# microsoft/MaskFlownet

Measured on NVIDIA H100. Metric: image-pairs/sec (MaskFlownet-S forward, 1024x448), higher is better.
Workload: dtype f32

## Files before the change

include/maskflow_b200.h:

```cpp
#ifndef MASKFLOW_B200_H_
#define MASKFLOW_B200_H_

#ifdef __cplusplus
extern "C" {
#endif

#define MFN_VERSION 100

#if defined(__GNUC__)
#define MFN_API __attribute__((visibility("default")))
#else
#define MFN_API
#endif

#define MFN_OK 0
#define MFN_ERR_INVALID_ARG (-1)
#define MFN_ERR_UNSUPPORTED (-2)
#define MFN_ERR_ALIGNMENT (-3)

#define MFN_CORR_AUTO 0
#define MFN_CORR_GENERIC 1
#define MFN_CORR_SIMT 2
#define MFN_CORR_MMA_BF16X3 3

#define MFN_BORDER_MXNET15 0
#define MFN_BORDER_ZERO_CORNER 1

MFN_API int mfn_version(void);
MFN_API const char* mfn_last_error(void);
MFN_API const char* mfn_last_kernel(void);
MFN_API unsigned long long mfn_launch_count(void);
MFN_API int mfn_set_tuning(const char* key, int value);

MFN_API int mfn_correlation_forward(const float* data1, const float* data2, float* out, int N, int C, int H,
                            int W, int pad_size, int kernel_size, int max_displacement, int stride1,
                            int stride2, int is_multiply, long long out_batch_stride,
                            float leaky_slope, int algo, void* stream);

MFN_API int mfn_correlation_backward(const float* grad_out, const float* out, const float* data1,
                             const float* data2, float* grad1, float* grad2, int N, int C, int H,
                             int W, int max_displacement, long long out_batch_stride,
                             float leaky_slope, void* stream);

MFN_API int mfn_deformable_conv_forward(const float* data, const float* offset, const float* weight,
                                const float* bias, float* out, int N, int C, int H, int W, int F,
                                int kernel_h, int kernel_w, int stride_h, int stride_w, int dilate_h,
                                int dilate_w, int pad_h, int pad_w, int num_group,
                                int num_deformable_group, int border_mode, void* stream);

MFN_API int mfn_deformable_conv_backward(const float* grad_out, const float* data, const float* offset,
                                 const float* weight, float* grad_data, float* grad_offset,
                                 float* grad_weight, float* grad_bias, int N, int C, int H, int W,
                                 int F, int border_mode, void* stream);

MFN_API int mfn_warp_mask_forward(const float* x, const float* flow_coarse, const float* mask_coarse,
                          const float* weight, const float* bias, const float* tradeoff, float* out,
                          float* flow_up_out, float* mask_up_out, float* conv_out, int N, int C,
                          int H, int W, int F, int upsample_factor, float flow_scale,
                          float level_stride, float leaky_slope, int border_mode, void* stream);

MFN_API int mfn_warp_mask_forward_tc(const float* x, const float* flow_coarse, const float* mask_coarse,
                                     const void* packed_weight, const float* bias, const float* tradeoff, float* out,
                                     float* flow_up_out, float* mask_up_out, float* conv_out, int N, int C, int H, int W,
                                     int F, int upsample_factor, float flow_scale, float level_stride, float leaky_slope,
                                     int border_mode, void* stream);

MFN_API long long mfn_warp_resample_workspace_bytes(int N, int F, int H, int W);
MFN_API int mfn_warp_mask_forward_resample(const float* x, const float* flow_coarse, const float* mask_coarse,
                                           const float* weight, const void* packed_weight, const float* bias,
                                           const float* tradeoff, void* workspace, float* out, float* flow_up_out,
                                           float* mask_up_out, int N, int C, int H, int W, int F, int upsample_factor,
                                           float flow_scale, float level_stride, float leaky_slope, int border_mode,
                                           void* stream);

MFN_API int mfn_warp_mask_backward(const float* grad_out, const float* out, const float* conv_out,
                           const float* x, const float* flow_up, const float* mask_up,
                           const float* weight, float* grad_x, float* grad_flow_up,
                           float* grad_mask_up, float* grad_weight, float* grad_bias,
                           float* grad_tradeoff, float* grad_conv_ws, int N, int C, int H, int W,
                           int F, float flow_scale, float level_stride, float leaky_slope,
                           int border_mode, void* stream);

MFN_API int mfn_upsample_forward(const float* in, float* out, int planes, int H, int W, int factor,
                         float scale, void* stream);
MFN_API int mfn_upsample_backward(const float* grad_out, float* grad_in, int planes, int H, int W, int factor,
                          float scale, void* stream);

MFN_API int mfn_grid_generator_warp_forward(const float* flow_xy, float* grid, int N, int H, int W,
                                    void* stream);
MFN_API int mfn_bilinear_sampler_forward(const float* data, const float* grid, float* out, int N, int C,
                                 int H, int W, int OH, int OW, void* stream);

MFN_API int mfn_grid_generator_warp_backward(const float* grad_grid, float* grad_flow, int N, int H, int W,
                                             void* stream);

MFN_API int mfn_bilinear_sampler_backward(const float* grad_out, const float* data, const float* grid,
                                          float* grad_data, float* grad_grid, int N, int C, int H, int W, int OH,
                                          int OW, void* stream);

MFN_API int mfn_image_warp_concat_forward(const float* im1, const float* im2, const float* flow_q,
                                  const float* mask_q, float* c30, float* c40, int N, int Ci, int H,
                                  int W, float flow_scale, void* stream);

MFN_API int mfn_image_warp_concat_backward(const float* grad_c40, const float* im2, const float* flow_q,
                                           const float* mask_q, float* grad_im2, float* grad_flow_up,
                                           float* grad_mask_up, int N, int Ci, int H, int W, float flow_scale,
                                           void* stream);

MFN_API long long mfn_conv3x3_packed_bytes(int Cin, int Cout);
MFN_API int mfn_conv3x3_pack_weights(const float* weight , void* packed, int Cin, int Cout,
                                     void* stream);
MFN_API int mfn_conv3x3_forward(const float* x, long long x_batch_stride, const void* packed_weight, const float* bias,
                                float* out, long long out_batch_stride, int N, int Cin, int H, int W, int Cout,
                                int dilation ,
                                float leaky_slope, void* stream);
#define MFN_CONV_OUT_NCHW 0
#define MFN_CONV_OUT_DEPTH_TO_SPACE2 1
#define MFN_CONV_OUT_LINEAR_PREFIX(k) ((k) << 8)
#define MFN_CONV_BF16 0x10
MFN_API int mfn_conv3x3_forward_ex(const float* x, long long x_batch_stride, const void* packed_weight, const float* bias,
                                   float* out, long long out_batch_stride, int N, int Cin, int H, int W, int Cout,
                                   int stride, int dilation, int out_mode, float leaky_slope, void* stream);
MFN_API long long mfn_conv3x3_workspace_bytes(int N, int Cin, int H, int W, int Cout, int stride, int dilation);
MFN_API int mfn_conv3x3_forward_ws(const float* x, long long x_batch_stride, const void* packed_weight, const float* bias,
                                   float* out, long long out_batch_stride, int N, int Cin, int H, int W, int Cout,
                                   int stride, int dilation, int out_mode, float leaky_slope, void* workspace,
                                   long long workspace_bytes, void* stream);

MFN_API int mfn_split_pack(const float* src, long long src_batch_stride, int N, int C, int H, int W, void* dst,
                           int dst_channels, int dst_c0, void* stream);
MFN_API int mfn_bf16_pack(const float* src, long long src_batch_stride, int N, int C, int H, int W, void* dst,
                          int dst_channels, int dst_c0, void* stream);
MFN_API int mfn_conv3x3_forward_split(const void* x, int x_channels, int x_c0, const void* packed_weight, const float* bias,
                                      float* out, long long out_batch_stride, void* out_split, int out_split_channels,
                                      int out_split_c0, int N, int Cin, int H, int W, int Cout, int dilation, int out_mode,
                                      float leaky_slope, void* workspace, long long workspace_bytes, void* stream);

MFN_API int mfn_preprocess_forward(const void* img1, const void* img2, int is_uint8, float* out1, float* out2,
                                   float* rgb_mean, int N, int C, int H, int W, int OH, int OW, void* stream);
MFN_API int mfn_postprocess_forward(const float* pred, float* out, int N, int channels, int Hq, int Wq, int H, int W,
                                    int flip_channels, int is_flow, void* stream);

MFN_API int mfn_flow_to_color(const float* flow_xy, unsigned char* rgb, float* rad_max, int N, int H, int W,
                              float max_radius, int bgr, void* stream);

MFN_API int mfn_flow_consistency(const float* flow_fw, const float* flow_bw, unsigned char* occ_fw, unsigned char* occ_bw,
                                 int N, int H, int W, float alpha, float beta, void* stream);

MFN_API long long mfn_interpolate_frames_workspace_bytes(int N, int H, int W);
MFN_API int mfn_interpolate_frames(const unsigned char* img0, const unsigned char* img1, const float* flow_fw,
                                   const float* flow_bw, const unsigned char* occ_fw, const unsigned char* occ_bw,
                                   unsigned char* out, void* ws, long long ws_bytes, int N, int H, int W,
                                   const float* times_host, int T, float occ_weight, void* stream);

MFN_API int mfn_warp_mask_backward_det(const float* grad_out, const float* out, const float* conv_out,
                                       const float* x, const float* flow_up, const float* mask_up,
                                       const float* weight, float* grad_x, float* grad_flow_up,
                                       float* grad_mask_up, float* grad_weight, float* grad_bias,
                                       float* grad_tradeoff, float* grad_conv_ws, int N, int C, int H, int W,
                                       int F, float flow_scale, float level_stride, float leaky_slope,
                                       int border_mode, void* det_ws, long long det_ws_bytes, void* stream);
MFN_API int mfn_deformable_conv_backward_det(const float* grad_out, const float* data, const float* offset,
                                             const float* weight, float* grad_data, float* grad_offset,
                                             float* grad_weight, float* grad_bias, int N, int C, int H, int W,
                                             int F, int border_mode, void* det_ws, long long det_ws_bytes,
                                             void* stream);
MFN_API int mfn_bilinear_sampler_backward_det(const float* grad_out, const float* data, const float* grid,
                                              float* grad_data, float* grad_grid, int N, int C, int H, int W,
                                              int OH, int OW, void* det_ws, long long det_ws_bytes, void* stream);
MFN_API int mfn_image_warp_concat_backward_det(const float* grad_c40, const float* im2, const float* flow_q,
                                               const float* mask_q, float* grad_im2, float* grad_flow_up,
                                               float* grad_mask_up, int N, int Ci, int H, int W, float flow_scale,
                                               void* det_ws, long long det_ws_bytes, void* stream);
MFN_API int mfn_preprocess_forward_det(const void* img1, const void* img2, int is_uint8, float* out1, float* out2,
                                       float* rgb_mean, int N, int C, int H, int W, int OH, int OW, void* det_ws,
                                       long long det_ws_bytes, void* stream);

MFN_API int mfn_geometry_augment_forward(const void* img1, const void* img2, int is_uint8, const float* flow, const void* mask,
                                         int mask_broadcast, const float* params, float* out_img1, float* out_img2,
                                         float* out_flow, float* out_mask, int N, int H, int W, int TH, int TW, void* stream);
MFN_API long long mfn_color_augment_workspace_bytes(int N);
MFN_API int mfn_color_augment_forward(const float* img1, const float* img2, const float* params, const float* noise1,
                                      const float* noise2, float noise_sigma, long long seed, float* out1, float* out2,
                                      void* workspace, long long workspace_bytes, int N, int H, int W, int has_gamma,
                                      void* stream);

MFN_API long long mfn_multiscale_epe_workspace_bytes(int N);
MFN_API int mfn_multiscale_epe_forward(const float* flow, const float* mask, const float* const* preds, const int* scales,
                                       const float* weights, int num_scales, float eps, float q, float* loss, float* mask_sum,
                                       void* workspace, long long workspace_bytes, int N, int H, int W, void* stream);
MFN_API int mfn_multiscale_epe_backward(const float* flow, const float* mask, const float* const* preds, const int* scales,
                                        const float* weights, int num_scales, float eps, float q, const float* grad_loss,
                                        const float* mask_sum, float* const* grad_preds, int N, int H, int W, void* stream);

MFN_API int mfn_census_loss_forward(const float* img1, const float* img2w, const unsigned char* occ, float* coef, float* vsum,
                                    float* loss, void* ws, long long ws_bytes, int N, int H, int W, void* stream);
MFN_API int mfn_census_loss_backward(const float* img1, const float* img2w, const float* coef, const float* vsum,
                                     const float* g_loss, float* g_img2w, int N, int H, int W, void* stream);
MFN_API int mfn_smoothness_loss_forward(const float* flow, const float* img, float* loss, void* ws, long long ws_bytes, int N,
                                        int H, int W, void* stream);
MFN_API int mfn_smoothness_loss_backward(const float* flow, const float* img, const float* g_loss, float* g_flow, int N,
                                         int H, int W, void* stream);

#ifdef __cplusplus
}
#endif
#endif
```

maskflownet_b200/_lib.py:

```python
from __future__ import annotations

import ctypes
import os
import subprocess

_HERE = os.path.dirname(os.path.abspath(__file__))
SO_PATH = os.environ.get("MFN_LIB_PATH") or os.path.join(_HERE, "libmaskflow_b200.so")
_lib = None

_f = ctypes.c_void_p
_i = ctypes.c_int
_ll = ctypes.c_longlong
_fl = ctypes.c_float

SIGNATURES = {
    "mfn_correlation_forward": [_f, _f, _f, _i, _i, _i, _i, _i, _i, _i, _i, _i, _i, _ll, _fl, _i, _f],
    "mfn_correlation_backward": [_f, _f, _f, _f, _f, _f, _i, _i, _i, _i, _i, _ll, _fl, _f],
    "mfn_deformable_conv_forward": [_f, _f, _f, _f, _f] + [_i] * 16 + [_f],
    "mfn_deformable_conv_backward": [_f] * 8 + [_i] * 6 + [_f],
    "mfn_warp_mask_forward": [_f] * 10 + [_i] * 6 + [_fl, _fl, _fl, _i, _f],
    "mfn_warp_mask_forward_tc": [_f] * 10 + [_i] * 6 + [_fl, _fl, _fl, _i, _f],
    "mfn_warp_mask_forward_resample": [_f] * 11 + [_i] * 6 + [_fl, _fl, _fl, _i, _f],
    "mfn_warp_mask_backward": [_f] * 14 + [_i] * 5 + [_fl, _fl, _fl, _i, _f],
    "mfn_upsample_forward": [_f, _f, _i, _i, _i, _i, _fl, _f],
    "mfn_upsample_backward": [_f, _f, _i, _i, _i, _i, _fl, _f],
    "mfn_grid_generator_warp_forward": [_f, _f, _i, _i, _i, _f],
    "mfn_bilinear_sampler_forward": [_f, _f, _f, _i, _i, _i, _i, _i, _i, _f],
    "mfn_image_warp_concat_forward": [_f] * 6 + [_i] * 4 + [_fl, _f],
    "mfn_grid_generator_warp_backward": [_f, _f, _i, _i, _i, _f],
    "mfn_bilinear_sampler_backward": [_f] * 5 + [_i] * 6 + [_f],
    "mfn_image_warp_concat_backward": [_f] * 7 + [_i] * 4 + [_fl, _f],
    "mfn_preprocess_forward": [_f, _f, _i, _f, _f, _f, _i, _i, _i, _i, _i, _i, _f],
    "mfn_postprocess_forward": [_f, _f, _i, _i, _i, _i, _i, _i, _i, _i, _f],
    "mfn_flow_to_color": [_f, _f, _f, _i, _i, _i, _fl, _i, _f],
    "mfn_flow_consistency": [_f, _f, _f, _f, _i, _i, _i, _fl, _fl, _f],
    "mfn_interpolate_frames_workspace_bytes": [_i, _i, _i],
    "mfn_interpolate_frames": [_f] * 8 + [_ll, _i, _i, _i, _f, _i, _fl, _f],
    "mfn_warp_mask_backward_det": [_f] * 14 + [_i] * 5 + [_fl, _fl, _fl, _i, _f, _ll, _f],
    "mfn_deformable_conv_backward_det": [_f] * 8 + [_i] * 6 + [_f, _ll, _f],
    "mfn_bilinear_sampler_backward_det": [_f] * 5 + [_i] * 6 + [_f, _ll, _f],
    "mfn_image_warp_concat_backward_det": [_f] * 7 + [_i] * 4 + [_fl, _f, _ll, _f],
    "mfn_preprocess_forward_det": [_f, _f, _i, _f, _f, _f, _i, _i, _i, _i, _i, _i, _f, _ll, _f],
    "mfn_geometry_augment_forward": [_f, _f, _i, _f, _f, _i, _f, _f, _f, _f, _f, _i, _i, _i, _i, _i, _f],
    "mfn_color_augment_forward": [_f, _f, _f, _f, _f, _fl, _ll, _f, _f, _f, _ll, _i, _i, _i, _i, _f],
    "mfn_multiscale_epe_forward": [_f, _f, _f, _f, _f, _i, _fl, _fl, _f, _f, _f, _ll, _i, _i, _i, _f],
    "mfn_multiscale_epe_backward": [_f, _f, _f, _f, _f, _i, _fl, _fl, _f, _f, _f, _i, _i, _i, _f],
    "mfn_census_loss_forward": [_f] * 7 + [_ll, _i, _i, _i, _f],
    "mfn_census_loss_backward": [_f] * 6 + [_i, _i, _i, _f],
    "mfn_smoothness_loss_forward": [_f] * 4 + [_ll, _i, _i, _i, _f],
    "mfn_smoothness_loss_backward": [_f] * 4 + [_i, _i, _i, _f],
    "mfn_set_tuning": [ctypes.c_char_p, _i],
    "mfn_conv3x3_pack_weights": [_f, _f, _i, _i, _f],
    "mfn_conv3x3_forward": [_f, _ll, _f, _f, _f, _ll, _i, _i, _i, _i, _i, _i, _fl, _f],
    "mfn_conv3x3_forward_ex": [_f, _ll, _f, _f, _f, _ll, _i, _i, _i, _i, _i, _i, _i, _i, _fl, _f],
    "mfn_conv3x3_forward_ws": [_f, _ll, _f, _f, _f, _ll, _i, _i, _i, _i, _i, _i, _i, _i, _fl, _f, _ll, _f],
    "mfn_conv3x3_forward_split": [_f, _i, _i, _f, _f, _f, _ll, _f, _i, _i] + [_i] * 7 + [_fl, _f, _ll, _f],
    "mfn_split_pack": [_f, _ll, _i, _i, _i, _i, _f, _i, _i, _f],
    "mfn_bf16_pack": [_f, _ll, _i, _i, _i, _i, _f, _i, _i, _f],
}
RESTYPES = {"mfn_interpolate_frames_workspace_bytes": _ll}


class MaskflowError(RuntimeError):
    pass


def build(verbose: bool = False) -> str:
    cmd = ["make", "-C", os.path.join(_HERE, "csrc"), "-j8"]
    res = subprocess.run(cmd, capture_output=not verbose, text=True)
    if res.returncode != 0:
        raise MaskflowError("building libmaskflow_b200.so failed:\n" + (res.stdout or "") + (res.stderr or ""))
    return SO_PATH


def lib() -> ctypes.CDLL:
    global _lib
    if _lib is None:
        if not os.path.exists(SO_PATH):
            raise MaskflowError(
                f"{SO_PATH} is missing: run `python -c 'import __graft_entry__ as g; g.build()'` "
                "(or `make -C maskflownet_b200/csrc`).  There is no CPU / PyTorch fallback for the hot path.")
        L = ctypes.CDLL(SO_PATH)
        L.mfn_version.restype = ctypes.c_int
        L.mfn_last_error.restype = ctypes.c_char_p
        L.mfn_last_kernel.restype = ctypes.c_char_p
        L.mfn_launch_count.restype = ctypes.c_ulonglong
        L.mfn_conv3x3_packed_bytes.restype = ctypes.c_longlong
        L.mfn_conv3x3_packed_bytes.argtypes = [ctypes.c_int, ctypes.c_int]
        L.mfn_conv3x3_workspace_bytes.restype = ctypes.c_longlong
        L.mfn_conv3x3_workspace_bytes.argtypes = [ctypes.c_int] * 7
        L.mfn_color_augment_workspace_bytes.restype = ctypes.c_longlong
        L.mfn_color_augment_workspace_bytes.argtypes = [ctypes.c_int]
        L.mfn_multiscale_epe_workspace_bytes.restype = ctypes.c_longlong
        L.mfn_multiscale_epe_workspace_bytes.argtypes = [ctypes.c_int]
        L.mfn_warp_resample_workspace_bytes.restype = ctypes.c_longlong
        L.mfn_warp_resample_workspace_bytes.argtypes = [ctypes.c_int] * 4
        for name, argtypes in SIGNATURES.items():
            fn = getattr(L, name)
            fn.argtypes = argtypes
            fn.restype = RESTYPES.get(name, ctypes.c_int)
        _lib = L
        for item in filter(None, os.environ.get("MFN_TUNING", "").split(",")):
            key, _, val = item.partition("=")
            if key.strip() in ("corr_dbg", "conv_dbg"):
                raise MaskflowError(f"MFN_TUNING: {key.strip()} is a profiling switch (results invalid); set it from a tool, "
                                    "not the environment")
            if L.mfn_set_tuning(key.strip().encode(), int(val)):
                raise MaskflowError(f"MFN_TUNING: {L.mfn_last_error().decode()}")
    return _lib


def last_error() -> str:
    return lib().mfn_last_error().decode()


def last_kernel() -> str:
    return lib().mfn_last_kernel().decode()


def launch_count() -> int:
    return int(lib().mfn_launch_count())


def call(name: str, *args) -> None:
    rc = getattr(lib(), name)(*args)
    if rc != 0:
        kind = "argument/support error" if rc < 0 else "CUDA error"
        raise MaskflowError(f"{name} failed ({kind} {rc}): {last_error()}")


def set_tuning(key: str, value: int) -> None:
    call("mfn_set_tuning", key.encode(), int(value))
```

maskflownet_b200/csrc/api.cu:

```cuda
#include <atomic>
#include <cstdarg>
#include <cstdio>
#include <cstring>

#include "common.cuh"

namespace mfn {

static thread_local char g_err[512] = "";
static thread_local const char* g_kernel = "";
static std::atomic<unsigned long long> g_launches{0};

int fail(int code, const char* fmt, ...) {
  va_list ap;
  va_start(ap, fmt);
  vsnprintf(g_err, sizeof(g_err), fmt, ap);
  va_end(ap);
  return code;
}

void note_kernel(const char* name) { g_kernel = name; }

Tuning& tuning() {
  static Tuning t;
  return t;
}

int check_launch(const char* kernel_name) {
  const cudaError_t e = cudaGetLastError();
  if (e != cudaSuccess) return fail((int)e, "%s: launch failed: %s", kernel_name, cudaGetErrorString(e));
  g_kernel = kernel_name;
  g_launches.fetch_add(1, std::memory_order_relaxed);
  g_err[0] = '\0';
  return MFN_OK;
}

}

extern "C" int mfn_version(void) { return MFN_VERSION; }
extern "C" const char* mfn_last_error(void) { return mfn::g_err; }
extern "C" const char* mfn_last_kernel(void) { return mfn::g_kernel; }
extern "C" unsigned long long mfn_launch_count(void) { return mfn::g_launches.load(std::memory_order_relaxed); }

extern "C" int mfn_set_tuning(const char* key, int value) {
  if (!key) return mfn::fail(MFN_ERR_INVALID_ARG, "mfn_set_tuning: null key");
  if (!strcmp(key, "corr_grid_cap")) mfn::tuning().corr_grid_cap = value;
  else if (!strcmp(key, "corr_disable_ring")) mfn::tuning().corr_disable_ring = value;
  else if (!strcmp(key, "warp_lin")) mfn::tuning().warp_lin = value;
  else if (!strcmp(key, "corr_rb")) mfn::tuning().corr_rb = value;
  else if (!strcmp(key, "warp_lin_fch")) mfn::tuning().warp_lin_fch = value;
  else if (!strcmp(key, "conv_as")) mfn::tuning().conv_as = value;
  else if (!strcmp(key, "conv_splitk")) mfn::tuning().conv_splitk = value;
  else if (!strcmp(key, "conv_narrow")) mfn::tuning().conv_narrow = value;
  else if (!strcmp(key, "conv_tma_in")) mfn::tuning().conv_tma_in = value;
  else if (!strcmp(key, "corr_rb_twb")) mfn::tuning().corr_rb_twb = value;
  else if (!strcmp(key, "corr_rb_rows")) mfn::tuning().corr_rb_rows = value;
  else if (!strcmp(key, "corr_tma")) mfn::tuning().corr_tma = value;
  else if (!strcmp(key, "corr_ts_lo")) mfn::tuning().corr_ts_lo = value;
  else if (!strcmp(key, "corr_ts_hi")) mfn::tuning().corr_ts_hi = value;
  else if (!strcmp(key, "corr_dbg")) mfn::tuning().corr_dbg = value;
  else if (!strcmp(key, "conv_dbg")) mfn::tuning().conv_dbg = value;
  else if (!strcmp(key, "corr_ring_th")) mfn::tuning().corr_ring_th = value;
  else if (!strcmp(key, "conv_wgmma")) mfn::tuning().conv_wgmma = value;
  else if (!strcmp(key, "conv_grid_cap")) mfn::tuning().conv_grid_cap = value;
  else if (!strcmp(key, "conv_wgmma_min_w")) mfn::tuning().conv_wgmma_min_w = value;
  else return mfn::fail(MFN_ERR_INVALID_ARG, "mfn_set_tuning: unknown key '%s'", key);
  return MFN_OK;
}
```

maskflownet_b200/csrc/common.cuh:

```cuda
#pragma once
#include <cuda_runtime.h>
#include <stdint.h>

#include "../../include/maskflow_b200.h"
#include "device_caps.h"
#include "sampling.cuh"

namespace mfn {

int fail(int code, const char* fmt, ...);
int check_launch(const char* kernel_name);
void note_kernel(const char* name);

struct Tuning {
  int corr_grid_cap = 0;
  int corr_disable_ring = 0;
  int conv_wgmma = 1;
  int conv_grid_cap = 0;
  int conv_wgmma_min_w = 1;
  int corr_ring_th = 8;
  int corr_rb = 1;
  int warp_lin_fch = 0;
  int conv_as = 0;
  int conv_splitk = 1;
  int conv_narrow = 1;
  int conv_tma_in = 1;
  int corr_rb_twb = 0;
  int corr_rb_rows = 0;
  int corr_tma = 1;
  int warp_lin = 1;
  int corr_ts_lo = 0, corr_ts_hi = 0;
  int corr_dbg = 0;
  int conv_dbg = 0;
};
Tuning& tuning();

static inline cudaStream_t as_stream(void* s) { return reinterpret_cast<cudaStream_t>(s); }

#define MFN_REQUIRE(cond, code, ...)                   \
  do {                                                 \
    if (!(cond)) return ::mfn::fail(code, __VA_ARGS__); \
  } while (0)

static inline bool aligned(const void* p, size_t a) { return (reinterpret_cast<uintptr_t>(p) % a) == 0; }

static inline unsigned grid_for(long long total, int threads) {
  long long b = (total + threads - 1) / threads;
  const long long cap = (long long)kNumSMs * 16;
  return (unsigned)(b < cap ? (b > 0 ? b : 1) : cap);
}


struct SmemOptIn {
  int bytes[64] = {};
};
template <typename K>
static inline cudaError_t ensure_dyn_smem(K kernel, int bytes, SmemOptIn& st) {
  int dev = 0;
  if (cudaGetDevice(&dev) != cudaSuccess) dev = -1;
  if (dev >= 0 && dev < 64 && st.bytes[dev] >= bytes) return cudaSuccess;
  const cudaError_t e = cudaFuncSetAttribute(kernel, cudaFuncAttributeMaxDynamicSharedMemorySize, bytes);
  if (e == cudaSuccess && dev >= 0 && dev < 64) st.bytes[dev] = bytes;
  return e;
}

long long warp_lin_workspace_bytes(int N, int F, int H, int W);
int launch_warp_lin(const float* x, const float* flow_c, const float* mask_c, const float* weight, const void* packed_weight,
                    const float* bias, const float* tradeoff, void* workspace, float* out, float* fup, float* mup, int N,
                    int C, int H, int W, int F, int up, float fs, float ls, float slope, int border_mode, cudaStream_t st);

int launch_corr_rb(int md, const float* d1, const float* d2, float* out, int N, int C, int H, int W, long long obs,
                   float slope, cudaStream_t st);

int launch_corr_tma(int md, const float* d1, const float* d2, float* out, int N, int C, int H, int W, long long obs,
                    float slope, cudaStream_t st);

int det_launch_abs_max(const float* v, long long n, unsigned* bound, cudaStream_t st);
int det_launch_pixel_abs_sum_max(const float* g, int N, int F, long long HW, unsigned* bound, cudaStream_t st);
int det_launch_fixed_to_float(const unsigned long long* acc, float* out, long long n, const unsigned* bound, int nb,
                              int fanin_bits, cudaStream_t st);
int det_launch_ordered_sum(const float* part, int nparts, long long part_stride, long long elem_stride, float* out,
                           long long n, int accumulate, cudaStream_t st);
int det_check_workspace(const char* fn, const void* ws, long long bytes, long long need);

__device__ __forceinline__ float leaky(float v, float slope) { return v > 0.f ? v : v * slope; }


struct Tap {
  int h0, h1, w0, w1;
  float lh, lw;
  bool valid;
  bool c00, c01, c10, c11;
};

template <int BORDER>
__device__ __forceinline__ Tap make_tap(float h, float w, int H, int W) {
  Tap t;
  if (BORDER == MFN_BORDER_MXNET15) {
    t.valid = (h >= 0.f) && (w >= 0.f) && (h < (float)H) && (w < (float)W);
    int h0 = (int)floorf(h), w0 = (int)floorf(w);
    if (h0 >= H - 1) {
      h0 = H - 1;
      t.h1 = h0;
      t.lh = 0.f;
    } else {
      t.h1 = h0 + 1;
      t.lh = h - (float)h0;
    }
    if (w0 >= W - 1) {
      w0 = W - 1;
      t.w1 = w0;
      t.lw = 0.f;
    } else {
      t.w1 = w0 + 1;
      t.lw = w - (float)w0;
    }
    t.h0 = h0;
    t.w0 = w0;
    if (!t.valid) {
      t.h0 = t.h1 = t.w0 = t.w1 = 0;
      t.lh = t.lw = 0.f;
    }
    t.c00 = t.c01 = t.c10 = t.c11 = t.valid;
  } else {
    t.valid = (h > -1.f) && (w > -1.f) && (h < (float)H) && (w < (float)W);
    const int h0 = (int)floorf(h), w0 = (int)floorf(w);
    t.lh = h - (float)h0;
    t.lw = w - (float)w0;
    const bool hin0 = h0 >= 0, hin1 = h0 + 1 <= H - 1, win0 = w0 >= 0, win1 = w0 + 1 <= W - 1;
    t.c00 = t.valid && hin0 && win0;
    t.c01 = t.valid && hin0 && win1;
    t.c10 = t.valid && hin1 && win0;
    t.c11 = t.valid && hin1 && win1;
    t.h0 = max(min(h0, H - 1), 0);
    t.h1 = max(min(h0 + 1, H - 1), 0);
    t.w0 = max(min(w0, W - 1), 0);
    t.w1 = max(min(w0 + 1, W - 1), 0);
    if (!t.valid) t.lh = t.lw = 0.f;
  }
  return t;
}

__device__ __forceinline__ float tap_sample(const Tap& t, const float* __restrict__ plane, int W) {
  const float hh = 1.f - t.lh, hw = 1.f - t.lw;
  float v = 0.f;
  if (t.c00) v += hh * hw * __ldg(plane + (size_t)t.h0 * W + t.w0);
  if (t.c01) v += hh * t.lw * __ldg(plane + (size_t)t.h0 * W + t.w1);
  if (t.c10) v += t.lh * hw * __ldg(plane + (size_t)t.h1 * W + t.w0);
  if (t.c11) v += t.lh * t.lw * __ldg(plane + (size_t)t.h1 * W + t.w1);
  return v;
}

}
```

maskflownet_b200/csrc/conv3x3.cu:

```cuda
#include "mma_tiles.cuh"

namespace mfn {
__global__ void conv3x3_pack_kernel(const float* __restrict__ w, unsigned char* __restrict__ packed, int Cin, int Cout,
                                    int CoutP, int nChunks) {
  using namespace c3;
  const long long total = (long long)nChunks * 9 * CoutP * 16;
  for (long long i = (long long)blockIdx.x * blockDim.x + threadIdx.x; i < total; i += (long long)gridDim.x * blockDim.x) {
    const int j = (int)(i & 15);
    const int f = (int)((i >> 4) % CoutP);
    const int tap = (int)((i / (16LL * CoutP)) % 9);
    const int q = (int)(i / (16LL * CoutP * 9));
    const int c = 32 * q + 2 * j;
    float a = 0.f, b = 0.f;
    if (f < Cout) {
      if (c < Cin) a = w[((size_t)f * Cin + c) * 9 + tap];
      if (c + 1 < Cin) b = w[((size_t)f * Cin + c + 1) * 9 + tap];
    }
    uint32_t hi, lo;
    split_pair(a, b, hi, lo);
    unsigned char* tile = packed + ((size_t)q * 9 + tap) * (2 * CoutP * PXB);
    const int off = swz(f, j >> 2) + (j & 3) * 4;
    *reinterpret_cast<uint32_t*>(tile + off) = hi;
    *reinterpret_cast<uint32_t*>(tile + CoutP * PXB + off) = lo;
  }
}

template <int WC, int NTN, bool PT>
__global__ void __launch_bounds__(c3::NTHREADS, 1)
    conv3x3_mma_kernel(const float* __restrict__ x, long long x_bs, const unsigned char* __restrict__ wpack,
                       const float* __restrict__ bias, float* __restrict__ out, long long out_bs, int Cin, int H, int W,
                       int Cout, int CoutP, int nChunks, float slope, int tilesX, int tilesY, int dil, int lin_prefix) {
  using namespace c3;
  constexpr int WR = 8 / WC;
  constexpr int TROWS = PT ? WR : WR + 2;
  constexpr int HWP = PT ? TW : c3::HWP;
  constexpr int IN_LO = TROWS * HWP * PXB;
  constexpr int IN_STAGE = 2 * IN_LO;
  const int WT_LO = CoutP * PXB;
  const int WT_BYTES = 2 * WT_LO;

  extern __shared__ __align__(128) unsigned char smem[];
  unsigned char* in_s = smem;
  unsigned char* wt_s = smem + 2 * IN_STAGE;

  const int tid = threadIdx.x, warp = tid >> 5, lane = tid & 31;
  const int wr = warp / WC, wc = warp % WC;
  const int tile = blockIdx.x;
  const int tx = tile % tilesX, ty = (tile / tilesX) % tilesY, n = tile / (tilesX * tilesY);
  const int x0 = tx * TW, y0 = ty * WR;
  const size_t plane = (size_t)H * W;
  const float* xn = x + (size_t)n * x_bs;

  constexpr int U_MAIN = TROWS * 4;
  constexpr int U_HALO = PT ? 0 : ((TROWS + 3) / 4) * 4;
  constexpr int U_TOT = U_MAIN + U_HALO;
  constexpr int UPW = (U_TOT + 7) / 8;
  auto unit_geom = [&](int u, int& row, int& chunk, int& pidx, int& xx, bool& act) {
    act = u < U_TOT;
    if (u < U_MAIN) {
      row = u >> 2;
      chunk = u & 3;
      pidx = PT ? lane : HX + lane;
      xx = x0 + lane;
    } else {
      const int k = u - U_MAIN;
      row = 4 * (k >> 2) + (lane >> 3);
      chunk = k & 3;
      const int px8 = lane & 7;
      pidx = px8 < 4 ? px8 : TW + px8;
      xx = px8 < 4 ? x0 - HX + px8 : x0 + TW + (px8 - 4);
      act = act && row < TROWS;
    }
  };
  auto load_tile = [&](int q, float (&e)[UPW][8]) {
    int sy = -1, sx = 0;
    if (PT) {
      const int tap = q % 9;
      sy = (tap / 3 - 1) * dil;
      sx = (tap % 3 - 1) * dil;
      q /= 9;
    }
#pragma unroll
    for (int k = 0; k < UPW; ++k) {
      int row, chunk, pidx, xx;
      bool act;
      unit_geom(warp * UPW + k, row, chunk, pidx, xx, act);
      xx += sx;
      const int yy = y0 + sy + row;
      const bool ok = act && yy >= 0 && yy < H && xx >= 0 && xx < W;
      const int c0 = 32 * q + 8 * chunk;
      const float* p = xn + (size_t)c0 * plane + (size_t)yy * W + xx;
#pragma unroll
      for (int c = 0; c < 8; ++c) {
        e[k][c] = (ok && c0 + c < Cin) ? __ldg(p) : 0.f;
        p += plane;
      }
    }
  };
  auto store_tile = [&](int stage, const float (&e)[UPW][8]) {
#pragma unroll
    for (int k = 0; k < UPW; ++k) {
      int row, chunk, pidx, xx;
      bool act;
      unit_geom(warp * UPW + k, row, chunk, pidx, xx, act);
      if (!act) continue;
      uint4 hi, lo;
      split_pair(e[k][0], e[k][1], hi.x, lo.x);
      split_pair(e[k][2], e[k][3], hi.y, lo.y);
      split_pair(e[k][4], e[k][5], hi.z, lo.z);
      split_pair(e[k][6], e[k][7], hi.w, lo.w);
      unsigned char* dst = in_s + stage * IN_STAGE + row * (HWP * PXB) + swz(pidx, chunk);
      *reinterpret_cast<uint4*>(dst) = hi;
      *reinterpret_cast<uint4*>(dst + IN_LO) = lo;
    }
  };
  auto load_weights = [&](int it, int stage) {
    const unsigned char* src = wpack + (size_t)it * WT_BYTES;
    const uint32_t dst = smem_u32(wt_s + stage * WT_BYTES);
    for (int o = tid * 16; o < WT_BYTES; o += NTHREADS * 16) cp_async16(dst + o, src + o);
  };

  const int g = lane >> 2, j = lane & 3;
  const int l8 = lane & 7, mi = lane >> 3;
  const int swB = (l8 >> 1) & 3;
  uint32_t offB[2];
#pragma unroll
  for (int kk = 0; kk < 2; ++kk) offB[kk] = (uint32_t)((8 * (mi >> 1) + l8) * PXB + (((2 * kk + (mi & 1)) ^ swB) << 4));
  const int fbase = wc * NTN * 8;

  float acc[2][NTN][4];
#pragma unroll
  for (int mt = 0; mt < 2; ++mt)
#pragma unroll
    for (int nt = 0; nt < NTN; ++nt)
#pragma unroll
      for (int i = 0; i < 4; ++i) acc[mt][nt][i] = 0.f;

  const int nIter = nChunks * 9;
  {
    float e[UPW][8];
    load_tile(0, e);
    store_tile(0, e);
  }
  load_weights(0, 0);
  cp_async_commit();
  if (nIter > 1) load_weights(1, 1);
  cp_async_commit();

  const uint32_t in_u32 = smem_u32(in_s), wt_u32 = smem_u32(wt_s);
  float pe[UPW][8];
  for (int it = 0; it < nIter; ++it) {
    const int q = it / 9, tap = it - 9 * q;
    const int ky = tap / 3, kx = tap - 3 * ky;
    cp_async_wait<1>();
    __syncthreads();
    if (it + 2 < nIter) load_weights(it + 2, (it + 2) % WSTAGES);
    cp_async_commit();
    if (PT) {
      if (it + 1 < nIter) load_tile(it + 1, pe);
    } else {
      if (tap == 0 && q + 1 < nChunks) load_tile(q + 1, pe);
      if (tap == 8 && q + 1 < nChunks) store_tile((q + 1) & 1, pe);
    }

    const uint32_t wst = wt_u32 + (uint32_t)((it % WSTAGES) * WT_BYTES);
    const uint32_t ist = PT ? in_u32 + (uint32_t)((it & 1) * IN_STAGE + wr * (HWP * PXB))
                            : in_u32 + (uint32_t)((q & 1) * IN_STAGE + (wr + ky) * (HWP * PXB));
    const bool half_chunk = 32 * q + 16 >= Cin;
#pragma unroll
    for (int kk = 0; kk < 2; ++kk) {
      if (kk == 1 && half_chunk) break;
      uint32_t ah[2][4], al[2][4];
#pragma unroll
      for (int mt = 0; mt < 2; ++mt) {
        const int p = (PT ? 0 : HX - 1 + kx) + 16 * mt + 8 * (mi & 1) + l8;
        const uint32_t a = ist + (uint32_t)(p * PXB + (((2 * kk + (mi >> 1)) ^ ((p >> 1) & 3)) << 4));
        ldsm_x4(a, ah[mt]);
        ldsm_x4(a + IN_LO, al[mt]);
      }
#pragma unroll
      for (int nt = 0; nt < NTN; nt += 2) {
        uint32_t bh[4], bl[4];
        const uint32_t b = wst + (uint32_t)((fbase + 8 * nt) * PXB) + offB[kk];
        ldsm_x4(b, bh);
        ldsm_x4(b + WT_LO, bl);
#pragma unroll
        for (int mt = 0; mt < 2; ++mt) {
          mma_bf16(acc[mt][nt], ah[mt], bl[0], bl[1]);
          mma_bf16(acc[mt][nt], al[mt], bh[0], bh[1]);
          mma_bf16(acc[mt][nt], ah[mt], bh[0], bh[1]);
          if (nt + 1 < NTN) {
            mma_bf16(acc[mt][nt + 1], ah[mt], bl[2], bl[3]);
            mma_bf16(acc[mt][nt + 1], al[mt], bh[2], bh[3]);
            mma_bf16(acc[mt][nt + 1], ah[mt], bh[2], bh[3]);
          }
        }
      }
    }
    if (PT && it + 1 < nIter) store_tile((it + 1) & 1, pe);
  }

  const int y = y0 + wr;
  if (y >= H) return;
  float* on = out + (size_t)n * out_bs + (size_t)y * W;
#pragma unroll
  for (int nt = 0; nt < NTN; ++nt) {
#pragma unroll
    for (int i = 0; i < 4; ++i) {
      const int f = fbase + 8 * nt + 2 * j + (i & 1);
      if (f >= Cout) continue;
      const float b = bias ? __ldg(bias + f) : 0.f;
#pragma unroll
      for (int mt = 0; mt < 2; ++mt) {
        const int xx = x0 + 16 * mt + g + 8 * (i >> 1);
        if (xx < W) on[(size_t)f * plane + xx] = leaky(acc[mt][nt][i] + b, f < lin_prefix ? 1.f : slope);
      }
    }
  }
}

template <int WC, int NTN, bool PT>
static int launch_conv_impl(const float* x, long long x_bs, const unsigned char* wpack, const float* bias, float* out,
                            long long out_bs, int N, int Cin, int H, int W, int Cout, int dil, float slope, int lin_prefix,
                            cudaStream_t st) {
  using namespace c3;
  constexpr int WR = 8 / WC;
  const int CoutP = cout_pad(Cout);
  const int nChunks = (Cin + 31) / 32;
  const int tilesX = (W + TW - 1) / TW, tilesY = (H + WR - 1) / WR;
  const int in_stage = PT ? 2 * WR * TW * PXB : 2 * (WR + 2) * HWP * PXB;
  const int smem = 2 * in_stage + WSTAGES * 2 * CoutP * PXB;
  static SmemOptIn opt;
  {
    const cudaError_t e = ensure_dyn_smem(conv3x3_mma_kernel<WC, NTN, PT>, smem, opt);
    if (e != cudaSuccess) return fail((int)e, "cudaFuncSetAttribute(conv3x3_mma_kernel): %s", cudaGetErrorString(e));
  }
  const unsigned grid = (unsigned)((long long)N * tilesX * tilesY);
  conv3x3_mma_kernel<WC, NTN, PT><<<grid, NTHREADS, smem, st>>>(x, x_bs, wpack, bias, out, out_bs, Cin, H, W, Cout,
                                                               CoutP, nChunks, slope, tilesX, tilesY, dil, lin_prefix);
  return check_launch(PT ? "conv3x3_mma_kernel<per-tap tiles>" : "conv3x3_mma_kernel<halo tile>");
}

template <int WC, int NTN>
static int launch_conv(const float* x, long long x_bs, const unsigned char* wpack, const float* bias, float* out,
                       long long out_bs, int N, int Cin, int H, int W, int Cout, int dil, float slope, int lin_prefix,
                       cudaStream_t st) {
  return dil == 1 ? launch_conv_impl<WC, NTN, false>(x, x_bs, wpack, bias, out, out_bs, N, Cin, H, W, Cout, 1, slope, lin_prefix, st)
                  : launch_conv_impl<WC, NTN, true>(x, x_bs, wpack, bias, out, out_bs, N, Cin, H, W, Cout, dil, slope, lin_prefix, st);
}

long long conv3x3_sync_packed_bytes(int Cin, int Cout) {
  if (Cout > 128) return 0;
  return (long long)((Cin + 31) / 32) * 9 * 2 * c3::cout_pad(Cout) * c3::PXB;
}

}

extern "C" long long mfn_conv3x3_packed_bytes(int Cin, int Cout) {
  if (Cin <= 0 || Cout <= 0) return 0;
  return mfn::conv3x3_sync_packed_bytes(Cin, Cout) + mfn::conv3x3_wgmma_packed_bytes(Cin, Cout);
}

extern "C" int mfn_conv3x3_pack_weights(const float* weight, void* packed, int Cin, int Cout, void* stream) {
  using namespace mfn;
  MFN_REQUIRE(weight && packed, MFN_ERR_INVALID_ARG, "mfn_conv3x3_pack_weights: null pointer");
  MFN_REQUIRE(Cin > 0 && Cout > 0, MFN_ERR_INVALID_ARG, "mfn_conv3x3_pack_weights: non-positive extent");
  MFN_REQUIRE(aligned(packed, 16), MFN_ERR_ALIGNMENT, "mfn_conv3x3_pack_weights: packed buffer must be 16-byte aligned");
  MFN_REQUIRE(Cout <= 256, MFN_ERR_UNSUPPORTED, "mfn_conv3x3_pack_weights: at most 256 output channels (got %d)", Cout);
  if (Cout <= 128) {
    const int CoutP = c3::cout_pad(Cout), nChunks = (Cin + 31) / 32;
    const long long total = (long long)nChunks * 9 * CoutP * 16;
    long long blocks = (total + 255) / 256;
    if (blocks > 4096) blocks = 4096;
    conv3x3_pack_kernel<<<(unsigned)blocks, 256, 0, as_stream(stream)>>>(weight, static_cast<unsigned char*>(packed), Cin,
                                                                         Cout, CoutP, nChunks);
    const int rc = check_launch("conv3x3_pack_kernel");
    if (rc) return rc;
  }
  return conv3x3_wgmma_pack(weight, static_cast<unsigned char*>(packed) + conv3x3_sync_packed_bytes(Cin, Cout), Cin, Cout,
                           as_stream(stream));
}

extern "C" int mfn_conv3x3_forward(const float* x, long long x_batch_stride, const void* packed_weight,
                                   const float* bias, float* out, long long out_batch_stride, int N, int Cin, int H,
                                   int W, int Cout, int dilation, float leaky_slope, void* stream) {
  return mfn_conv3x3_forward_ex(x, x_batch_stride, packed_weight, bias, out, out_batch_stride, N, Cin, H, W, Cout, 1,
                                dilation, MFN_CONV_OUT_NCHW, leaky_slope, stream);
}

extern "C" int mfn_conv3x3_forward_ex(const float* x, long long x_batch_stride, const void* packed_weight,
                                      const float* bias, float* out, long long out_batch_stride, int N, int Cin, int H,
                                      int W, int Cout, int stride, int dilation, int out_mode, float leaky_slope,
                                      void* stream) {
  return mfn_conv3x3_forward_ws(x, x_batch_stride, packed_weight, bias, out, out_batch_stride, N, Cin, H, W, Cout, stride,
                                dilation, out_mode, leaky_slope, nullptr, 0, stream);
}

extern "C" long long mfn_conv3x3_workspace_bytes(int N, int Cin, int H, int W, int Cout, int stride, int dilation) {
  using namespace mfn;
  if (N <= 0 || Cin <= 0 || H <= 0 || W <= 0 || Cout <= 0 || Cout > 256 || dilation < 1 ||
      !(stride == 1 || (stride == 2 && dilation == 1)))
    return 0;
  if (!(tuning().conv_wgmma && W >= tuning().conv_wgmma_min_w) && Cout <= 128 && stride == 1) return 0;
  return conv3x3_wgmma_workspace_bytes(N, Cin, H, W, Cout, stride, dilation);
}

extern "C" int mfn_conv3x3_forward_ws(const float* x, long long x_batch_stride, const void* packed_weight,
                                      const float* bias, float* out, long long out_batch_stride, int N, int Cin, int H,
                                      int W, int Cout, int stride, int dilation, int out_mode, float leaky_slope,
                                      void* workspace, long long workspace_bytes, void* stream) {
  using namespace mfn;
  MFN_REQUIRE(workspace_bytes >= 0 && (workspace || workspace_bytes == 0) && aligned(workspace, 16), MFN_ERR_INVALID_ARG,
              "mfn_conv3x3_forward_ws: workspace must be 16-byte aligned (or null with 0 bytes)");
  MFN_REQUIRE(x && packed_weight && out, MFN_ERR_INVALID_ARG, "mfn_conv3x3_forward: null pointer");
  MFN_REQUIRE(N > 0 && Cin > 0 && H > 0 && W > 0 && Cout > 0, MFN_ERR_INVALID_ARG,
              "mfn_conv3x3_forward: non-positive extent");
  MFN_REQUIRE(Cout <= 256, MFN_ERR_UNSUPPORTED, "mfn_conv3x3_forward: at most 256 output channels (got %d)", Cout);
  MFN_REQUIRE(dilation >= 1, MFN_ERR_INVALID_ARG, "mfn_conv3x3_forward: dilation must be >= 1");
  MFN_REQUIRE(stride == 1 || (stride == 2 && dilation == 1), MFN_ERR_UNSUPPORTED,
              "mfn_conv3x3_forward: stride must be 1, or 2 with dilation 1 (got stride %d, dilation %d)", stride, dilation);
  MFN_REQUIRE(aligned(packed_weight, 16), MFN_ERR_ALIGNMENT, "mfn_conv3x3_forward: packed weights must be 16-byte aligned");
  const int bf16 = out_mode & MFN_CONV_BF16;
  out_mode &= ~MFN_CONV_BF16;
  const int lin_prefix = out_mode >> 8, mode = out_mode & 0xff;
  MFN_REQUIRE(mode == MFN_CONV_OUT_NCHW || (mode == MFN_CONV_OUT_DEPTH_TO_SPACE2 && stride == 1 && Cout % 4 == 0),
              MFN_ERR_INVALID_ARG, "mfn_conv3x3_forward: depth-to-space output needs stride 1 and Cout %% 4 == 0");
  MFN_REQUIRE(lin_prefix >= 0 && lin_prefix <= Cout && (lin_prefix == 0 || mode == MFN_CONV_OUT_NCHW), MFN_ERR_INVALID_ARG,
              "mfn_conv3x3_forward: linear prefix (out_mode >> 8 = %d) needs NCHW output and <= Cout", lin_prefix);
  const int OH = (H - 1) / stride + 1, OW = (W - 1) / stride + 1;
  const long long xbs = x_batch_stride ? x_batch_stride : (long long)Cin * H * W;
  const long long obs = out_batch_stride ? out_batch_stride : (long long)Cout * OH * OW;
  MFN_REQUIRE(xbs >= (long long)Cin * H * W && obs >= (long long)Cout * OH * OW, MFN_ERR_INVALID_ARG,
              "mfn_conv3x3_forward: batch stride smaller than the tensor");
  const unsigned char* wp = static_cast<const unsigned char*>(packed_weight);
  cudaStream_t st = as_stream(stream);
  const bool sync_ok = Cout <= 128 && stride == 1 && mode == MFN_CONV_OUT_NCHW;
  if ((tuning().conv_wgmma && W >= tuning().conv_wgmma_min_w) || !sync_ok) {
    const int rc = conv3x3_wgmma_launch(x, xbs, wp + conv3x3_sync_packed_bytes(Cin, Cout), bias, out, obs, N, Cin, H, W,
                                       Cout, stride, dilation, out_mode | bf16, leaky_slope, st, 0,
                                       static_cast<float*>(workspace), workspace_bytes);
    if (rc != -1) return rc;
    MFN_REQUIRE(sync_ok, MFN_ERR_UNSUPPORTED, "mfn_conv3x3_forward: shape fits neither kernel (Cout=%d stride=%d dilation=%d)",
                Cout, stride, dilation);
  }
  MFN_REQUIRE(!bf16, MFN_ERR_UNSUPPORTED,
              "mfn_conv3x3_forward: MFN_CONV_BF16 runs on the wgmma kernel only, and this launch would take the mma.sync "
              "kernel (tuning conv_wgmma = 0, or W = %d < conv_wgmma_min_w)", W);
  const int nt = (Cout + 7) / 8;
  if (nt <= 4) return launch_conv<1, 4>(x, xbs, wp, bias, out, obs, N, Cin, H, W, Cout, dilation, leaky_slope, lin_prefix, st);
  if (nt <= 8) return launch_conv<1, 8>(x, xbs, wp, bias, out, obs, N, Cin, H, W, Cout, dilation, leaky_slope, lin_prefix, st);
  if (nt <= 12) return launch_conv<2, 6>(x, xbs, wp, bias, out, obs, N, Cin, H, W, Cout, dilation, leaky_slope, lin_prefix, st);
  return launch_conv<2, 8>(x, xbs, wp, bias, out, obs, N, Cin, H, W, Cout, dilation, leaky_slope, lin_prefix, st);
}

extern "C" int mfn_conv3x3_forward_split(const void* x, int x_channels, int x_c0, const void* packed_weight,
                                         const float* bias, float* out, long long out_batch_stride, void* out_split,
                                         int out_split_channels, int out_split_c0, int N, int Cin, int H, int W, int Cout,
                                         int dilation, int out_mode, float leaky_slope, void* workspace,
                                         long long workspace_bytes, void* stream) {
  using namespace mfn;
  MFN_REQUIRE(workspace_bytes >= 0 && (workspace || workspace_bytes == 0) && aligned(workspace, 16), MFN_ERR_INVALID_ARG,
              "mfn_conv3x3_forward_split: workspace must be 16-byte aligned (or null with 0 bytes)");
  const int bf16 = out_mode & MFN_CONV_BF16;
  out_mode &= ~MFN_CONV_BF16;
  const int lin_prefix = out_mode >> 8, mode = out_mode & 0xff;
  MFN_REQUIRE(x && packed_weight && (out || (out_split && lin_prefix == 0)), MFN_ERR_INVALID_ARG,
              "mfn_conv3x3_forward_split: null pointer");
  MFN_REQUIRE(N > 0 && Cin > 0 && H > 0 && W > 0 && Cout > 0 && Cout <= 256 && dilation >= 1, MFN_ERR_INVALID_ARG,
              "mfn_conv3x3_forward_split: bad extent, Cout (<= 256) or dilation");
  MFN_REQUIRE(x_c0 >= 0 && x_c0 % 16 == 0 && x_c0 + Cin <= x_channels &&
                  ((x_c0 + Cin) % 16 == 0 || x_c0 + Cin == x_channels),
              MFN_ERR_INVALID_ARG,
              "mfn_conv3x3_forward_split: input slice [%d, %d) of the %d channels must start at a multiple of 16 and end "
              "at one or at the last channel", x_c0, x_c0 + Cin, x_channels);
  MFN_REQUIRE(aligned(packed_weight, 16) && aligned(x, 16), MFN_ERR_ALIGNMENT,
              "mfn_conv3x3_forward_split: packed weights and split input must be 16-byte aligned");
  MFN_REQUIRE(lin_prefix >= 0 && lin_prefix <= Cout && (lin_prefix == 0 || mode == MFN_CONV_OUT_NCHW), MFN_ERR_INVALID_ARG,
              "mfn_conv3x3_forward_split: linear prefix needs NCHW / split output and <= Cout");
  MFN_REQUIRE(mode == MFN_CONV_OUT_NCHW || (mode == MFN_CONV_OUT_DEPTH_TO_SPACE2 && Cout % 4 == 0 && !out_split),
              MFN_ERR_INVALID_ARG, "mfn_conv3x3_forward_split: depth-to-space output needs Cout %% 4 == 0 and fp32 output");
  const int Fo = out_split ? lin_prefix : (mode ? Cout / 4 : Cout), OS = mode ? 4 : 1;
  const long long obs = out_batch_stride ? out_batch_stride : (long long)Fo * H * W * OS;
  MFN_REQUIRE(obs >= (long long)Fo * H * W * OS, MFN_ERR_INVALID_ARG, "mfn_conv3x3_forward_split: batch stride too small");
  SplitIO sio;
  sio.in = x;
  sio.in_C = x_channels;
  sio.in_c0 = x_c0;
  sio.out = out_split;
  sio.out_C = out_split_channels;
  sio.out_c0 = out_split_c0;
  const unsigned char* wp = static_cast<const unsigned char*>(packed_weight);
  const int rc = conv3x3_wgmma_launch(nullptr, 0, wp + conv3x3_sync_packed_bytes(Cin, Cout), bias, out, obs, N, Cin, H, W,
                                      Cout, 1, dilation, out_mode | bf16, leaky_slope, as_stream(stream), 0,
                                      static_cast<float*>(workspace), workspace_bytes, sio);
  MFN_REQUIRE(rc != -1, MFN_ERR_UNSUPPORTED,
              "mfn_conv3x3_forward_split: unsupported (odd dilation >= 2, split output slice not 16-channel aligned "
              "after an even linear prefix, or too large)");
  return rc;
}
```

maskflownet_b200/csrc/conv3x3_wgmma.cu:

```cuda
#include <cstring>
#include <type_traits>

#include "mma_tiles.cuh"
#include "split_act.cuh"

namespace mfn {
namespace um {
constexpr int MT_WIDE = 128, MT_NARROW = 64;
inline int tile_width(int OW, int stride) {
  return tuning().conv_narrow && (OW <= MT_NARROW || (stride == 2 && tuning().conv_tma_in)) ? MT_NARROW : MT_WIDE;
}
constexpr int R = 2;
constexpr int NTHREADS = 384;
constexpr int NCONS = 8;
constexpr int NPROD = 3;
constexpr int MAX_AS = 4, MAX_WS = 24;
constexpr int MAX_RS = 4;
constexpr int BATCH = 6;
constexpr int BAR_BYTES = 1024;

__host__ __device__ inline int n_slots(int stride, int dil) { return stride == 2 ? 2 * R + 1 : (dil >= R ? 3 * R : R + 2 * dil); }
__host__ __device__ inline int row_pitch(int mt, int stride, int dil) { return stride == 2 ? 2 * mt + 1 : mt + 2 * dil; }
__host__ __device__ inline int slot_of(int r, int ky, int stride, int dil) {
  return stride == 2 ? 2 * r + ky : (dil >= R ? ky * R + r : r + ky * dil);
}
__host__ __device__ inline int tap_xoff(int mt, int kx, int stride, int dil) {
  return stride == 2 ? (kx == 1 ? 0 : (kx == 0 ? mt : mt + 1)) : kx * dil;
}
__host__ __device__ inline int band_map(int v, int n) { return v < n ? v : (v == n + 2 ? 0 : (v == n + 5 ? n - 1 : -1)); }
__host__ __device__ inline int raw_pitch(int mt, int stride) { return stride == 2 ? 2 * mt + 4 : mt + 8; }
__host__ __device__ inline int raw_channels(int stride) { return stride == 2 ? 8 : 16; }
__host__ __device__ inline int raw_stage_bytes(int nslots, int mt, int stride) {
  return raw_channels(stride) * nslots * raw_pitch(mt, stride) * 4;
}
__host__ __device__ inline int raw_ring_max(int stride) { return stride == 2 ? MAX_RS : 2; }
__host__ __device__ inline int cout_pad(int cout) { return cout <= 128 ? (cout + 15) / 16 * 16 : 256; }
__host__ __device__ inline bool fold_hi_lo(int CoutP) { return CoutP <= 64; }
__host__ __device__ inline int taps_per_stage(int CoutP) { return CoutP <= 32 ? 9 : (CoutP <= 64 ? 3 : 1); }

__device__ __forceinline__ uint64_t desc_hi(uint32_t lbo_bytes, uint32_t sbo_bytes) {
  return ((uint64_t)((lbo_bytes >> 4) & 0x3FFFu) << 16) | ((uint64_t)((sbo_bytes >> 4) & 0x3FFFu) << 32);
}
__device__ __forceinline__ void wgmma_fence() { asm volatile("wgmma.fence.sync.aligned;" ::: "memory"); }
__device__ __forceinline__ void wgmma_commit() { asm volatile("wgmma.commit_group.sync.aligned;" ::: "memory"); }
template <int N>
__device__ __forceinline__ void wgmma_wait() { asm volatile("wgmma.wait_group.sync.aligned %0;" ::"n"(N) : "memory"); }
template <int S>
__device__ __forceinline__ void fence_acc(float (&d)[S]) {
#pragma unroll
  for (int i = 0; i < S; ++i) asm volatile("" : "+f"(d[i])::"memory");
}
template <int S>
__device__ __forceinline__ void wgmma_n16(float (&d)[S], uint64_t a, uint64_t b, uint32_t scale_d) {
  static_assert(S >= 8, "accumulator too small");
  asm volatile(
      "{\n\t.reg .pred p;\n\tsetp.ne.b32 p, %10, 0;\n\t"
      "wgmma.mma_async.sync.aligned.m64n16k16.f32.bf16.bf16 {%0, %1, %2, %3, %4, %5, %6, %7}, %8, %9, p, 1, 1, 0, 0;\n\t}"
      : "+f"(d[0]), "+f"(d[1]), "+f"(d[2]), "+f"(d[3]), "+f"(d[4]), "+f"(d[5]), "+f"(d[6]), "+f"(d[7])
      : "l"(a), "l"(b), "r"(scale_d));
}
template <int S>
__device__ __forceinline__ void wgmma_n32(float (&d)[S], uint64_t a, uint64_t b, uint32_t scale_d) {
  static_assert(S >= 16, "accumulator too small");
  asm volatile(
      "{\n\t.reg .pred p;\n\tsetp.ne.b32 p, %18, 0;\n\t"
      "wgmma.mma_async.sync.aligned.m64n32k16.f32.bf16.bf16 {%0, %1, %2, %3, %4, %5, %6, %7, %8, %9, %10, %11, %12, %13, %14, %15}, %16, %17, p, 1, 1, 0, 0;\n\t}"
      : "+f"(d[0]), "+f"(d[1]), "+f"(d[2]), "+f"(d[3]), "+f"(d[4]), "+f"(d[5]), "+f"(d[6]), "+f"(d[7]), "+f"(d[8]), "+f"(d[9]), "+f"(d[10]), "+f"(d[11]), "+f"(d[12]), "+f"(d[13]), "+f"(d[14]), "+f"(d[15])
      : "l"(a), "l"(b), "r"(scale_d));
}
template <int S>
__device__ __forceinline__ void wgmma_n48(float (&d)[S], uint64_t a, uint64_t b, uint32_t scale_d) {
  static_assert(S >= 24, "accumulator too small");
  asm volatile(
      "{\n\t.reg .pred p;\n\tsetp.ne.b32 p, %26, 0;\n\t"
      "wgmma.mma_async.sync.aligned.m64n48k16.f32.bf16.bf16 {%0, %1, %2, %3, %4, %5, %6, %7, %8, %9, %10, %11, %12, %13, %14, %15, %16, %17, %18, %19, %20, %21, %22, %23}, %24, %25, p, 1, 1, 0, 0;\n\t}"
      : "+f"(d[0]), "+f"(d[1]), "+f"(d[2]), "+f"(d[3]), "+f"(d[4]), "+f"(d[5]), "+f"(d[6]), "+f"(d[7]), "+f"(d[8]), "+f"(d[9]), "+f"(d[10]), "+f"(d[11]), "+f"(d[12]), "+f"(d[13]), "+f"(d[14]), "+f"(d[15]), "+f"(d[16]), "+f"(d[17]), "+f"(d[18]), "+f"(d[19]), "+f"(d[20]), "+f"(d[21]), "+f"(d[22]), "+f"(d[23])
      : "l"(a), "l"(b), "r"(scale_d));
}
template <int S>
__device__ __forceinline__ void wgmma_n64(float (&d)[S], uint64_t a, uint64_t b, uint32_t scale_d) {
  static_assert(S >= 32, "accumulator too small");
  asm volatile(
      "{\n\t.reg .pred p;\n\tsetp.ne.b32 p, %34, 0;\n\t"
      "wgmma.mma_async.sync.aligned.m64n64k16.f32.bf16.bf16 {%0, %1, %2, %3, %4, %5, %6, %7, %8, %9, %10, %11, %12, %13, %14, %15, %16, %17, %18, %19, %20, %21, %22, %23, %24, %25, %26, %27, %28, %29, %30, %31}, %32, %33, p, 1, 1, 0, 0;\n\t}"
      : "+f"(d[0]), "+f"(d[1]), "+f"(d[2]), "+f"(d[3]), "+f"(d[4]), "+f"(d[5]), "+f"(d[6]), "+f"(d[7]), "+f"(d[8]), "+f"(d[9]), "+f"(d[10]), "+f"(d[11]), "+f"(d[12]), "+f"(d[13]), "+f"(d[14]), "+f"(d[15]), "+f"(d[16]), "+f"(d[17]), "+f"(d[18]), "+f"(d[19]), "+f"(d[20]), "+f"(d[21]), "+f"(d[22]), "+f"(d[23]), "+f"(d[24]), "+f"(d[25]), "+f"(d[26]), "+f"(d[27]), "+f"(d[28]), "+f"(d[29]), "+f"(d[30]), "+f"(d[31])
      : "l"(a), "l"(b), "r"(scale_d));
}
template <int S>
__device__ __forceinline__ void wgmma_n80(float (&d)[S], uint64_t a, uint64_t b, uint32_t scale_d) {
  static_assert(S >= 40, "accumulator too small");
  asm volatile(
      "{\n\t.reg .pred p;\n\tsetp.ne.b32 p, %42, 0;\n\t"
      "wgmma.mma_async.sync.aligned.m64n80k16.f32.bf16.bf16 {%0, %1, %2, %3, %4, %5, %6, %7, %8, %9, %10, %11, %12, %13, %14, %15, %16, %17, %18, %19, %20, %21, %22, %23, %24, %25, %26, %27, %28, %29, %30, %31, %32, %33, %34, %35, %36, %37, %38, %39}, %40, %41, p, 1, 1, 0, 0;\n\t}"
      : "+f"(d[0]), "+f"(d[1]), "+f"(d[2]), "+f"(d[3]), "+f"(d[4]), "+f"(d[5]), "+f"(d[6]), "+f"(d[7]), "+f"(d[8]), "+f"(d[9]), "+f"(d[10]), "+f"(d[11]), "+f"(d[12]), "+f"(d[13]), "+f"(d[14]), "+f"(d[15]), "+f"(d[16]), "+f"(d[17]), "+f"(d[18]), "+f"(d[19]), "+f"(d[20]), "+f"(d[21]), "+f"(d[22]), "+f"(d[23]), "+f"(d[24]), "+f"(d[25]), "+f"(d[26]), "+f"(d[27]), "+f"(d[28]), "+f"(d[29]), "+f"(d[30]), "+f"(d[31]), "+f"(d[32]), "+f"(d[33]), "+f"(d[34]), "+f"(d[35]), "+f"(d[36]), "+f"(d[37]), "+f"(d[38]), "+f"(d[39])
      : "l"(a), "l"(b), "r"(scale_d));
}
template <int S>
__device__ __forceinline__ void wgmma_n96(float (&d)[S], uint64_t a, uint64_t b, uint32_t scale_d) {
  static_assert(S >= 48, "accumulator too small");
  asm volatile(
      "{\n\t.reg .pred p;\n\tsetp.ne.b32 p, %50, 0;\n\t"
      "wgmma.mma_async.sync.aligned.m64n96k16.f32.bf16.bf16 {%0, %1, %2, %3, %4, %5, %6, %7, %8, %9, %10, %11, %12, %13, %14, %15, %16, %17, %18, %19, %20, %21, %22, %23, %24, %25, %26, %27, %28, %29, %30, %31, %32, %33, %34, %35, %36, %37, %38, %39, %40, %41, %42, %43, %44, %45, %46, %47}, %48, %49, p, 1, 1, 0, 0;\n\t}"
      : "+f"(d[0]), "+f"(d[1]), "+f"(d[2]), "+f"(d[3]), "+f"(d[4]), "+f"(d[5]), "+f"(d[6]), "+f"(d[7]), "+f"(d[8]), "+f"(d[9]), "+f"(d[10]), "+f"(d[11]), "+f"(d[12]), "+f"(d[13]), "+f"(d[14]), "+f"(d[15]), "+f"(d[16]), "+f"(d[17]), "+f"(d[18]), "+f"(d[19]), "+f"(d[20]), "+f"(d[21]), "+f"(d[22]), "+f"(d[23]), "+f"(d[24]), "+f"(d[25]), "+f"(d[26]), "+f"(d[27]), "+f"(d[28]), "+f"(d[29]), "+f"(d[30]), "+f"(d[31]), "+f"(d[32]), "+f"(d[33]), "+f"(d[34]), "+f"(d[35]), "+f"(d[36]), "+f"(d[37]), "+f"(d[38]), "+f"(d[39]), "+f"(d[40]), "+f"(d[41]), "+f"(d[42]), "+f"(d[43]), "+f"(d[44]), "+f"(d[45]), "+f"(d[46]), "+f"(d[47])
      : "l"(a), "l"(b), "r"(scale_d));
}
template <int S>
__device__ __forceinline__ void wgmma_n112(float (&d)[S], uint64_t a, uint64_t b, uint32_t scale_d) {
  static_assert(S >= 56, "accumulator too small");
  asm volatile(
      "{\n\t.reg .pred p;\n\tsetp.ne.b32 p, %58, 0;\n\t"
      "wgmma.mma_async.sync.aligned.m64n112k16.f32.bf16.bf16 {%0, %1, %2, %3, %4, %5, %6, %7, %8, %9, %10, %11, %12, %13, %14, %15, %16, %17, %18, %19, %20, %21, %22, %23, %24, %25, %26, %27, %28, %29, %30, %31, %32, %33, %34, %35, %36, %37, %38, %39, %40, %41, %42, %43, %44, %45, %46, %47, %48, %49, %50, %51, %52, %53, %54, %55}, %56, %57, p, 1, 1, 0, 0;\n\t}"
      : "+f"(d[0]), "+f"(d[1]), "+f"(d[2]), "+f"(d[3]), "+f"(d[4]), "+f"(d[5]), "+f"(d[6]), "+f"(d[7]), "+f"(d[8]), "+f"(d[9]), "+f"(d[10]), "+f"(d[11]), "+f"(d[12]), "+f"(d[13]), "+f"(d[14]), "+f"(d[15]), "+f"(d[16]), "+f"(d[17]), "+f"(d[18]), "+f"(d[19]), "+f"(d[20]), "+f"(d[21]), "+f"(d[22]), "+f"(d[23]), "+f"(d[24]), "+f"(d[25]), "+f"(d[26]), "+f"(d[27]), "+f"(d[28]), "+f"(d[29]), "+f"(d[30]), "+f"(d[31]), "+f"(d[32]), "+f"(d[33]), "+f"(d[34]), "+f"(d[35]), "+f"(d[36]), "+f"(d[37]), "+f"(d[38]), "+f"(d[39]), "+f"(d[40]), "+f"(d[41]), "+f"(d[42]), "+f"(d[43]), "+f"(d[44]), "+f"(d[45]), "+f"(d[46]), "+f"(d[47]), "+f"(d[48]), "+f"(d[49]), "+f"(d[50]), "+f"(d[51]), "+f"(d[52]), "+f"(d[53]), "+f"(d[54]), "+f"(d[55])
      : "l"(a), "l"(b), "r"(scale_d));
}
template <int S>
__device__ __forceinline__ void wgmma_n128(float (&d)[S], uint64_t a, uint64_t b, uint32_t scale_d) {
  static_assert(S >= 64, "accumulator too small");
  asm volatile(
      "{\n\t.reg .pred p;\n\tsetp.ne.b32 p, %66, 0;\n\t"
      "wgmma.mma_async.sync.aligned.m64n128k16.f32.bf16.bf16 {%0, %1, %2, %3, %4, %5, %6, %7, %8, %9, %10, %11, %12, %13, %14, %15, %16, %17, %18, %19, %20, %21, %22, %23, %24, %25, %26, %27, %28, %29, %30, %31, %32, %33, %34, %35, %36, %37, %38, %39, %40, %41, %42, %43, %44, %45, %46, %47, %48, %49, %50, %51, %52, %53, %54, %55, %56, %57, %58, %59, %60, %61, %62, %63}, %64, %65, p, 1, 1, 0, 0;\n\t}"
      : "+f"(d[0]), "+f"(d[1]), "+f"(d[2]), "+f"(d[3]), "+f"(d[4]), "+f"(d[5]), "+f"(d[6]), "+f"(d[7]), "+f"(d[8]), "+f"(d[9]), "+f"(d[10]), "+f"(d[11]), "+f"(d[12]), "+f"(d[13]), "+f"(d[14]), "+f"(d[15]), "+f"(d[16]), "+f"(d[17]), "+f"(d[18]), "+f"(d[19]), "+f"(d[20]), "+f"(d[21]), "+f"(d[22]), "+f"(d[23]), "+f"(d[24]), "+f"(d[25]), "+f"(d[26]), "+f"(d[27]), "+f"(d[28]), "+f"(d[29]), "+f"(d[30]), "+f"(d[31]), "+f"(d[32]), "+f"(d[33]), "+f"(d[34]), "+f"(d[35]), "+f"(d[36]), "+f"(d[37]), "+f"(d[38]), "+f"(d[39]), "+f"(d[40]), "+f"(d[41]), "+f"(d[42]), "+f"(d[43]), "+f"(d[44]), "+f"(d[45]), "+f"(d[46]), "+f"(d[47]), "+f"(d[48]), "+f"(d[49]), "+f"(d[50]), "+f"(d[51]), "+f"(d[52]), "+f"(d[53]), "+f"(d[54]), "+f"(d[55]), "+f"(d[56]), "+f"(d[57]), "+f"(d[58]), "+f"(d[59]), "+f"(d[60]), "+f"(d[61]), "+f"(d[62]), "+f"(d[63])
      : "l"(a), "l"(b), "r"(scale_d));
}
template <int N, int S>
__device__ __forceinline__ void wgmma_bf16(float (&d)[S], uint64_t a, uint64_t b, uint32_t scale_d) {
  if constexpr (N == 16) wgmma_n16(d, a, b, scale_d);
  else if constexpr (N == 32) wgmma_n32(d, a, b, scale_d);
  else if constexpr (N == 48) wgmma_n48(d, a, b, scale_d);
  else if constexpr (N == 64) wgmma_n64(d, a, b, scale_d);
  else if constexpr (N == 80) wgmma_n80(d, a, b, scale_d);
  else if constexpr (N == 96) wgmma_n96(d, a, b, scale_d);
  else if constexpr (N == 112) wgmma_n112(d, a, b, scale_d);
  else wgmma_n128(d, a, b, scale_d);
}

struct SplitK {
  int k, from, n_lo, y_lo, rh;
  long long part_stride;
  float* ws;
  uint32_t magic_tp, magic_tx;
  int as_wide;
  int ns;
  int stg;
};
__device__ __forceinline__ void decode_tile(int tile, int tilesX, int tilesY, const SplitK& sk, int& tx, int& ty, int& n) {
  if (sk.magic_tp) {
    n = (int)__umulhi((uint32_t)tile, sk.magic_tp);
    const int rem = tile - n * tilesX * tilesY;
    ty = sk.magic_tx ? (int)__umulhi((uint32_t)rem, sk.magic_tx) : rem;
    tx = rem - ty * tilesX;
  } else {
    tx = tile % tilesX;
    ty = (tile / tilesX) % tilesY;
    n = tile / (tilesX * tilesY);
  }
}
struct SplitDev {
  int in, in_g0, in_Cg;
  unsigned char* out;
  int out_Cg, out_c0;
};
struct Work {
  int tile, part, cb, ce, nh;
};
__device__ __forceinline__ Work decode_work(int w, const SplitK& sk, int nChunks) {
  Work r;
  r.nh = 0;
  if (sk.ns == 2) {
    r.nh = w & 1;
    w >>= 1;
  }
  if (sk.k <= 1 || w < sk.from) {
    r.tile = w; r.part = -1; r.cb = 0; r.ce = nChunks;
  } else {
    const int u = w - sk.from, t = u / sk.k;
    r.tile = sk.from + t;
    r.part = u - t * sk.k;
    r.cb = r.part * nChunks / sk.k;
    r.ce = (r.part + 1) * nChunks / sk.k;
  }
  return r;
}

struct SmemMap {
  int a_lo, a_stage, w_tile, w_stage, w_off, bar_off, stg_off, total, AS, WS, raw_off, raw_stage, RS;
};
constexpr int STG_CH = 32, SPITCH = MT_WIDE + 4;
constexpr int STG_BYTES = R * STG_CH * SPITCH * 4;
__host__ __device__ inline SmemMap smem_map(int E, int CoutP, int as_wide = 3, int stg = 0, int terms = 3, int raw = 0,
                                            int rs_max = 2) {
  SmemMap m;
  m.a_lo = 2 * E * 16;
  m.a_stage = terms == 1 ? m.a_lo : 2 * m.a_lo;
  m.w_tile = terms == 1 ? 32 * CoutP : 64 * CoutP;
  int budget = 227 * 1024 - BAR_BYTES - stg;
  m.w_stage = taps_per_stage(CoutP) * m.w_tile;
  m.RS = 0;
  if (raw) {
    const int raw_off = (2 * m.a_stage + 127) / 128 * 128;
    m.RS = rs_max;
    while (m.RS > 2 && budget - raw_off - m.RS * raw < 3 * m.w_stage) --m.RS;
    budget -= m.RS * raw + (raw_off - 2 * m.a_stage);
  }
  if (raw)
    m.AS = 2;
  else if (taps_per_stage(CoutP) > 1)
    m.AS = (4 * m.a_stage + 4 * m.w_stage <= budget) ? 4 : ((3 * m.a_stage + 3 * m.w_stage <= budget) ? 3 : 2);
  else
    m.AS = (as_wide >= 3 && 3 * m.a_stage + 8 * m.w_stage <= budget) ? 3 : 2;
  int ws = (budget - m.AS * m.a_stage) / m.w_stage;
  m.WS = ws > MAX_WS ? MAX_WS : ws;
  m.raw_off = raw ? (m.AS * m.a_stage + 127) / 128 * 128 : m.AS * m.a_stage;
  m.raw_stage = raw;
  m.w_off = m.raw_off + m.RS * raw;
  m.bar_off = m.w_off + m.WS * m.w_stage;
  m.stg_off = m.bar_off + BAR_BYTES;
  m.total = m.stg_off + stg;
  return m;
}
}

__global__ void conv3x3_pack_wgmma_kernel(const float* __restrict__ w, unsigned char* __restrict__ packed, int Cin, int Cout,
                                          int CoutP, int nChunks16) {
  const long long total = (long long)nChunks16 * 9 * CoutP * 8;
  for (long long i = (long long)blockIdx.x * blockDim.x + threadIdx.x; i < total; i += (long long)gridDim.x * blockDim.x) {
    const int j = (int)(i & 7);
    const int f = (int)((i >> 3) % CoutP);
    const int tap = (int)((i / (8LL * CoutP)) % 9);
    const int c = (int)(i / (8LL * CoutP * 9));
    const int ch = 16 * c + 2 * j;
    float a = 0.f, b = 0.f;
    if (f < Cout) {
      if (ch < Cin) a = w[((size_t)f * Cin + ch) * 9 + tap];
      if (ch + 1 < Cin) b = w[((size_t)f * Cin + ch + 1) * 9 + tap];
    }
    uint32_t hi, lo;
    split_pair(a, b, hi, lo);
    const int wt = 64 * CoutP;
    unsigned char* tile = packed + ((size_t)c * 9 + tap) * wt;
    if (um::fold_hi_lo(CoutP)) {
      const int off = (j >> 2) * (2 * CoutP * 16) + f * 16 + (j & 3) * 4;
      *reinterpret_cast<uint32_t*>(tile + off) = hi;
      *reinterpret_cast<uint32_t*>(tile + CoutP * 16 + off) = lo;
    } else {
      const int off = (j >> 2) * (CoutP * 16) + f * 16 + (j & 3) * 4;
      *reinterpret_cast<uint32_t*>(tile + off) = hi;
      *reinterpret_cast<uint32_t*>(tile + wt / 2 + off) = lo;
    }
  }
}

template <int NW, bool FOLD, int TPS, int TERMS, int MT>
__global__ void __launch_bounds__(um::NTHREADS, 1)
    conv3x3_wgmma_kernel(const float* __restrict__ x, long long x_bs, const unsigned char* __restrict__ wpack,
                         const float* __restrict__ bias_arg, float* __restrict__ out_base, long long out_bs, int Cin, int H, int W,
                         int OH, int OW, int Cout, int CoutP, int nChunks, float slope_arg, int tilesX, int tilesY, int numWork,
                         int stride, int dil, int out_mode_arg, int ext, um::SplitK sk, um::SplitDev xs,
                         const __grid_constant__ CUtensorMap tmx, int dbg) {
  using namespace um;
  static_assert(TERMS == 1 || TERMS == 3, "one or three products per multiply-add");
  static_assert(MT == MT_WIDE || MT == MT_NARROW, "128- or 64-pixel tile rows");
  constexpr bool FOLD_ACC = FOLD && TERMS == 3;
  constexpr int P = TERMS == 1 ? 1 : 2;
  constexpr int NCOL = FOLD_ACC ? NW / 2 : NW;
  constexpr int MB = MT / 64;
  const int out_mode_k = out_mode_arg & 0xff, lin_prefix_k = out_mode_arg >> 8;
  extern __shared__ __align__(128) unsigned char smem[];
  const int nslots = n_slots(stride, dil), PW = row_pitch(MT, stride, dil), E = nslots * PW;
  const SmemMap sm = smem_map(E, CoutP, sk.as_wide, sk.stg, TERMS, xs.in == 2 ? raw_stage_bytes(nslots, MT, stride) : 0,
                              raw_ring_max(stride));
  const int AS = sm.AS, WS = sm.WS, RS = sm.RS;
  const uint32_t s_base = smem_u32(smem);
  const uint32_t bar0 = s_base + sm.bar_off;
  const uint32_t a_full = bar0, a_empty = bar0 + 8 * MAX_AS, w_full = bar0 + 16 * MAX_AS, w_empty = w_full + 8 * MAX_WS;
  const uint32_t r_full = w_empty + 8 * MAX_WS, r_empty = r_full + 8 * MAX_RS;

  const int tid = threadIdx.x, lane = tid & 31;
  const int warp = __shfl_sync(0xffffffffu, tid >> 5, 0);
  const size_t plane = (size_t)H * W;

  if (tid == 0) {
    for (int i = 0; i < AS; ++i) {
      mbar_init(a_full + 8 * i, xs.in == 1 ? 1 : NPROD);
      mbar_init(a_empty + 8 * i, NCONS);
    }
    for (int i = 0; i < RS; ++i) {
      mbar_init(r_full + 8 * i, 1);
      mbar_init(r_empty + 8 * i, NPROD);
    }
    for (int i = 0; i < WS; ++i) {
      mbar_init(w_full + 8 * i, 1);
      mbar_init(w_empty + 8 * i, NCONS);
    }
    asm volatile("fence.mbarrier_init.release.cluster;" ::: "memory");
  }
  __syncthreads();

  if (warp < 8) {
    const int r = warp >> 2, wq = warp & 3;
    const uint32_t a_lbo = (uint32_t)E * 16u, b_lbo = (uint32_t)(FOLD_ACC ? 2 * CoutP : CoutP) * 16u;
    uint32_t a_off[9];
#pragma unroll
    for (int tap = 0; tap < 9; ++tap)
      a_off[tap] = (uint32_t)(slot_of(r, tap / 3, stride, dil) * PW + tap_xoff(MT, tap % 3, stride, dil));
    const uint64_t dh_a = desc_hi(a_lbo, 128u), dh_b = desc_hi(b_lbo, 128u);
    uint32_t as = 0, aph = 0, ws = 0, wph = 0;
    const uint32_t a_lo16 = (uint32_t)sm.a_lo >> 4, a_stage16 = (uint32_t)sm.a_stage >> 4, s_base16 = s_base >> 4;
    const uint32_t w_base16 = (s_base + (uint32_t)sm.w_off) >> 4, w_tile16 = (uint32_t)sm.w_tile >> 4, w_half16 = w_tile16 >> 1;
    const uint32_t w_stage16 = (uint32_t)sm.w_stage >> 4;
    int rel_w = -1, rel_a = -1;
    auto release = [&]() {
      if (lane == 0) {
        if (rel_w >= 0) mbar_arrive(w_empty + 8 * rel_w);
        if (rel_a >= 0) mbar_arrive(a_empty + 8 * rel_a);
      }
      rel_w = rel_a = -1;
    };
    float acc[MB][NW / 2];
    for (int work = blockIdx.x; work < numWork; work += gridDim.x) {
      const Work wk = decode_work(work, sk, nChunks);
      const int cb = wk.cb, ce = wk.ce;
      const uint32_t b_nh16 = (uint32_t)(wk.nh * NCOL);
#pragma unroll
      for (int mh = 0; mh < MB; ++mh) fence_acc(acc[mh]);
      if (dbg & 8) {
        for (int c = cb; c < ce; ++c) {
          mbar_wait(a_full + 8 * as, aph);
          for (int tap = 0; tap < 9; ++tap) {
            if (tap % TPS == 0) mbar_wait(w_full + 8 * ws, wph);
            release();
            if (tap % TPS == TPS - 1) {
              rel_w = (int)ws;
              if (++ws == (uint32_t)WS) { ws = 0; wph ^= 1; }
            }
            if (tap == 8) rel_a = (int)as;
          }
          if (++as == (uint32_t)AS) { as = 0; aph ^= 1; }
        }
      }
      for (int c = (dbg & 8) ? ce : cb; c < ce; ++c) {
        mbar_wait(a_full + 8 * as, aph);
        const uint32_t a_st16 = s_base16 + as * a_stage16;
#pragma unroll
        for (int tap = 0; tap < 9; ++tap) {
          if (tap % TPS == 0) mbar_wait(w_full + 8 * ws, wph);
          const uint32_t w16 = w_base16 + ws * w_stage16 + (uint32_t)(tap % TPS) * w_tile16 + b_nh16;
          const uint64_t b_hi = dh_b | (uint64_t)w16, b_lo = dh_b | (uint64_t)(w16 + w_half16);
          const uint32_t sc = (tap == 0 && c == cb) ? 0u : 1u;
          wgmma_fence();
#pragma unroll
          for (int mh = 0; mh < MB; ++mh) {
            const uint32_t a16 = a_st16 + a_off[tap] + (uint32_t)(64 * mh);
            const uint64_t a_hi = dh_a | (uint64_t)a16, a_lo = dh_a | (uint64_t)(a16 + a_lo16);
            if constexpr (TERMS == 1) {
              wgmma_bf16<NW>(acc[mh], a_hi, b_hi, sc);
            } else if constexpr (FOLD) {
              wgmma_bf16<NW>(acc[mh], a_hi, b_hi, sc);
              wgmma_bf16<NW / 2>(acc[mh], a_lo, b_hi, 1u);
            } else {
              wgmma_bf16<NW>(acc[mh], a_hi, b_lo, sc);
              wgmma_bf16<NW>(acc[mh], a_lo, b_hi, 1u);
              wgmma_bf16<NW>(acc[mh], a_hi, b_hi, 1u);
            }
          }
          wgmma_commit();
          wgmma_wait<1>();
          release();
          if (tap % TPS == TPS - 1) {
            rel_w = (int)ws;
            if (++ws == (uint32_t)WS) { ws = 0; wph ^= 1; }
          }
          if (tap == 8) rel_a = (int)as;
        }
        if (++as == (uint32_t)AS) { as = 0; aph ^= 1; }
      }
      wgmma_wait<0>();
#pragma unroll
      for (int mh = 0; mh < MB; ++mh) fence_acc(acc[mh]);
      release();

      int tx, ty, n;
      decode_tile(wk.tile, tilesX, tilesY, sk, tx, ty, n);
      const bool partial = wk.part >= 0;
      const float* const bias = partial ? nullptr : bias_arg;
      const float slope = partial ? 1.f : slope_arg;
      const int out_mode = partial ? 0 : out_mode_k, lin_prefix = partial ? 0 : lin_prefix_k;
      const size_t oplane0 = partial ? (size_t)sk.rh * OW : (size_t)OH * OW;
      float* const out = partial ? sk.ws + (size_t)wk.part * (size_t)sk.part_stride + (size_t)(n - sk.n_lo) * Cout * oplane0 -
                                       (size_t)sk.y_lo * OW
                                 : out_base + (size_t)n * out_bs;
      const int y = ty * R + r;
      const int F = Cout >> 2;
      const size_t oplane2 = (size_t)(2 * OH) * (2 * OW);
      if (y < OH && !(dbg & 4) && sk.stg && !partial) {
        constexpr int SCH = NCOL % STG_CH == 0 ? STG_CH : 16;
        float* const stg = reinterpret_cast<float*>(smem + sm.stg_off) + r * STG_CH * SPITCH;
        const int t = wq * 32 + lane;
        const int x0 = tx * MT;
        const uint32_t seg = (uint32_t)((OW - x0 < MT ? OW - x0 : MT) * 4);
        if (xs.out != nullptr) {
          unsigned char* const sst = reinterpret_cast<unsigned char*>(stg);
#pragma unroll
          for (int pc = 0; pc < NCOL / SCH; ++pc) {
            if (t < SCH * P / 8) bulk_wait_read();
            named_bar_sync(1 + r, 128);
#pragma unroll
            for (int jj = 0; jj < SCH / 8; ++jj) {
              const int j = pc * (SCH / 8) + jj;
              const int f = wk.nh * NCOL + 8 * j + 2 * (lane & 3);
              const float b0 = (bias != nullptr && f < Cout) ? __ldg(bias + f) : 0.f;
              const float b1 = (bias != nullptr && f + 1 < Cout) ? __ldg(bias + f + 1) : 0.f;
              unsigned char* const row = sst + (P * jj * MT + 16 * wq + (lane >> 2)) * 16 + (lane & 3) * 4;
#pragma unroll
              for (int mh = 0; mh < MB; ++mh)
#pragma unroll
                for (int h = 0; h < 2; ++h) {
                  const int i = 4 * j + 2 * h;
                  float v0 = acc[mh][i], v1 = acc[mh][i + 1];
                  if constexpr (FOLD_ACC) {
                    v0 += acc[mh][i + NW / 4];
                    v1 += acc[mh][i + 1 + NW / 4];
                  }
                  unsigned char* const e = row + (64 * mh + 8 * h) * 16;
                  if constexpr (TERMS == 1) {
                    *reinterpret_cast<uint32_t*>(e) = bf16_pair(leaky(v0 + b0, slope), leaky(v1 + b1, slope));
                  } else {
                    uint32_t hi, lo;
                    split_pair(leaky(v0 + b0, slope), leaky(v1 + b1, slope), hi, lo);
                    *reinterpret_cast<uint32_t*>(e) = hi;
                    *reinterpret_cast<uint32_t*>(e + MT * 16) = lo;
                  }
                }
            }
            asm volatile("fence.proxy.async.shared::cta;" ::: "memory");
            named_bar_sync(1 + r, 128);
            const int f = wk.nh * NCOL + pc * SCH + 8 * (t >> (P - 1));
            if (t < SCH * P / 8 && f < Cout) {
              const long long dst = sa::entry<P>(n, t & (P - 1), (xs.out_c0 + f) >> 3, (long long)y * OW + x0, xs.out_Cg,
                                                 oplane0);
              bulk_s2g(xs.out + dst, smem_u32(sst + t * MT * 16), seg * 4);
              bulk_commit();
            }
          }
        } else
#pragma unroll
        for (int pc = 0; pc < NCOL / SCH; ++pc) {
          if (t < SCH) bulk_wait_read();
          named_bar_sync(1 + r, 128);
#pragma unroll
          for (int jj = 0; jj < SCH / 8; ++jj) {
            const int j = pc * (SCH / 8) + jj;
#pragma unroll
            for (int e = 0; e < 2; ++e) {
              const int f = wk.nh * NCOL + 8 * j + 2 * (lane & 3) + e;
              const float b = (bias != nullptr && f < Cout) ? __ldg(bias + f) : 0.f;
              const float sl = f < lin_prefix ? 1.f : slope;
              float* const row = stg + (8 * jj + 2 * (lane & 3) + e) * SPITCH + 16 * wq + (lane >> 2);
#pragma unroll
              for (int mh = 0; mh < MB; ++mh)
#pragma unroll
                for (int h = 0; h < 2; ++h) {
                  const int i = 4 * j + 2 * h + e;
                  float v = acc[mh][i];
                  if constexpr (FOLD_ACC) v += acc[mh][i + NW / 4];
                  row[64 * mh + 8 * h] = leaky(v + b, sl);
                }
            }
          }
          asm volatile("fence.proxy.async.shared::cta;" ::: "memory");
          named_bar_sync(1 + r, 128);
          const int f = wk.nh * NCOL + pc * SCH + t;
          if (t < SCH && f < Cout) {
            bulk_s2g(out + (size_t)f * oplane0 + (size_t)y * OW + x0, smem_u32(stg + t * SPITCH), seg);
            bulk_commit();
          }
        }
      } else if (y < OH && !(dbg & 4)) {
#pragma unroll
        for (int mh = 0; mh < MB; ++mh) {
#pragma unroll
          for (int h = 0; h < 2; ++h) {
            const int xx = tx * MT + 64 * mh + 16 * wq + (lane >> 2) + 8 * h;
            if (xx >= OW) continue;
#pragma unroll
            for (int j = 0; j < NCOL / 8; ++j) {
#pragma unroll
              for (int e = 0; e < 2; ++e) {
                const int i = 4 * j + 2 * h + e;
                float v = acc[mh][i];
                if constexpr (FOLD_ACC) v += acc[mh][i + NW / 4];
                const int f = wk.nh * NCOL + 8 * j + 2 * (lane & 3) + e;
                if (f >= Cout) continue;
                if (xs.out != nullptr && !partial && f >= lin_prefix) {
                  if (e == 0) {
                    const float b0 = bias != nullptr ? __ldg(bias + f) : 0.f, b1 = bias != nullptr ? __ldg(bias + f + 1) : 0.f;
                    float v1 = acc[mh][i + 1];
                    if constexpr (FOLD_ACC) v1 += acc[mh][i + 1 + NW / 4];
                    sa::put_pair<P>(xs.out, xs.out_Cg, oplane0, n, xs.out_c0 + f - lin_prefix, (size_t)y * OW + xx,
                                 leaky(v + b0, slope), leaky(v1 + b1, slope));
                  }
                } else if (out_mode == 0) {
                  const float t = v + (bias != nullptr ? __ldg(bias + f) : 0.f);
                  out[(size_t)f * oplane0 + (size_t)y * OW + xx] = leaky(t, f < lin_prefix ? 1.f : slope);
                } else {
                  const int ph = f / F, ff = f - ph * F;
                  const float t = v + (bias != nullptr ? __ldg(bias + ff) : 0.f);
                  out[(size_t)ff * oplane2 + (size_t)(2 * y + (ph >> 1)) * (2 * OW) + 2 * xx + (ph & 1)] = leaky(t, slope);
                }
              }
            }
          }
        }
      }
    }
    bulk_wait_all();
  } else if (warp == 8) {
    if (lane == 0) {
      uint32_t ws = 0, wph = 0;
      bool wrapped = false;
      for (int work = blockIdx.x; work < numWork; work += gridDim.x) {
        const Work wk = decode_work(work, sk, nChunks);
        const int cb = wk.cb, ce = wk.ce;
        if constexpr (TERMS == 3) {
          const unsigned char* src = wpack + (size_t)cb * 9 * sm.w_tile;
          for (int it = 9 * cb; it < 9 * ce; it += TPS, src += sm.w_stage) {
            if (wrapped) mbar_wait(w_empty + 8 * ws, wph ^ 1);
            mbar_arrive_expect_tx(w_full + 8 * ws, (uint32_t)sm.w_stage);
            bulk_g2s(s_base + (uint32_t)sm.w_off + ws * (uint32_t)sm.w_stage, src, (uint32_t)sm.w_stage, w_full + 8 * ws);
            if (++ws == (uint32_t)WS) { ws = 0; wph ^= 1; wrapped = true; }
          }
        } else {
          const int gt = 64 * CoutP, run = 16 * CoutP;
          const unsigned char* src = wpack + (size_t)cb * 9 * gt;
          for (int it = 9 * cb; it < 9 * ce; it += TPS, src += TPS * gt) {
            if (wrapped) mbar_wait(w_empty + 8 * ws, wph ^ 1);
            mbar_arrive_expect_tx(w_full + 8 * ws, (uint32_t)sm.w_stage);
            const uint32_t dst = s_base + (uint32_t)sm.w_off + ws * (uint32_t)sm.w_stage;
#pragma unroll 1
            for (int t = 0; t < TPS; ++t) {
              if constexpr (FOLD) {
                bulk_g2s(dst + (uint32_t)(t * sm.w_tile), src + t * gt, (uint32_t)run, w_full + 8 * ws);
                bulk_g2s(dst + (uint32_t)(t * sm.w_tile + run), src + t * gt + 2 * run, (uint32_t)run, w_full + 8 * ws);
              } else {
                bulk_g2s(dst + (uint32_t)(t * sm.w_tile), src + t * gt, (uint32_t)sm.w_tile, w_full + 8 * ws);
              }
            }
            if (++ws == (uint32_t)WS) { ws = 0; wph ^= 1; wrapped = true; }
          }
        }
      }
    }
  } else {
    if (xs.in == 1) {
      if (warp == 9 && lane == 0) {
        uint32_t as = 0, aph = 0;
        bool wrapped = false;
        for (int work = blockIdx.x; work < numWork; work += gridDim.x) {
          const Work wk = decode_work(work, sk, nChunks);
          int tx, ty, n;
          decode_tile(wk.tile, tilesX, tilesY, sk, tx, ty, n);
          const int x0 = tx * MT - dil, y0 = ty * R;
          const int gb = n * P * xs.in_Cg + xs.in_g0;
          for (int c = wk.cb; c < wk.ce; ++c) {
            if (wrapped) mbar_wait(a_empty + 8 * as, aph ^ 1);
            const uint32_t bar = a_full + 8 * as, dst = s_base + as * (uint32_t)sm.a_stage;
            if (dbg & 16) {
              mbar_arrive(bar);
            } else {
              mbar_arrive_expect_tx(bar, (uint32_t)sm.a_stage);
              const int g = gb + 2 * c;
              if (dil < R) {
                tma_load_4d(dst, &tmx, 0, x0, y0 - dil, g, bar);
                if constexpr (P == 2) tma_load_4d(dst + (uint32_t)sm.a_lo, &tmx, 0, x0, y0 - dil, g + xs.in_Cg, bar);
              } else if constexpr (P == 1) {
#pragma unroll 1
                for (int k = 0; k < 6; ++k) {
                  const int ky = k >> 1, kc = k & 1;
                  tma_load_4d(dst + (uint32_t)((kc * E + ky * R * PW) * 16), &tmx, 0, x0, y0 + (ky - 1) * dil, g + kc, bar);
                }
              } else {
#pragma unroll 1
                for (int k = 0; k < 12; ++k) {
                  const int ky = k >> 2, kc = (k >> 1) & 1, pl = k & 1;
                  tma_load_4d(dst + (uint32_t)(pl * sm.a_lo + (kc * E + ky * R * PW) * 16), &tmx, 0, x0, y0 + (ky - 1) * dil,
                              g + kc + pl * xs.in_Cg, bar);
                }
              }
            }
            if (++as == (uint32_t)AS) { as = 0; aph ^= 1; wrapped = true; }
          }
        }
      }
      return;
    }
    if (dbg & 16) {
      uint32_t as = 0, aph = 0;
      bool wrapped = false;
      for (int work = blockIdx.x; work < numWork; work += gridDim.x) {
        const Work wk = decode_work(work, sk, nChunks);
        for (int c = wk.cb; c < wk.ce; ++c) {
          if (wrapped) mbar_wait(a_empty + 8 * as, aph ^ 1);
          __syncwarp();
          if (lane == 0) mbar_arrive(a_full + 8 * as);
          if (++as == (uint32_t)AS) { as = 0; aph ^= 1; wrapped = true; }
        }
      }
      return;
    }
    const int pw = warp - 9;
    const int G = (E + 31) / 32;
    const bool one_plane = Cin <= 8;
    const int nItems = one_plane ? G : 2 * G;
    const int nb = (nItems + NPROD * BATCH - 1) / (NPROD * BATCH);
    const uint32_t pw_magic = 0xFFFFFFFFu / (uint32_t)PW + 1u;
    if (one_plane) {
      for (int st = 0; st < AS; ++st)
        for (int e = pw * 32 + lane; e < E; e += NPROD * 32) {
          unsigned char* d = smem + st * sm.a_stage + (E + e) * 16;
          *reinterpret_cast<uint4*>(d) = make_uint4(0u, 0u, 0u, 0u);
          if constexpr (P == 2) *reinterpret_cast<uint4*>(d + sm.a_lo) = make_uint4(0u, 0u, 0u, 0u);
        }
    }
    if (xs.in == 2) {
      const bool s2 = stride == 2;
      const int RP = raw_pitch(MT, stride), CP = nslots * RP;
      const int RPC = s2 && !one_plane ? 2 : 1;
      const uint32_t raw_bytes = (uint32_t)sm.raw_stage, raw_base = s_base + (uint32_t)sm.raw_off;
      const bool issuer = warp == 9 && lane == 0;
      int i_work = blockIdx.x, i_c = 0, i_h = 0, i_ce = 0, i_x = 0, i_y = 0, i_n = 0;
      auto i_tile = [&]() {
        if (i_work >= numWork) return;
        const Work wk = decode_work(i_work, sk, nChunks);
        int tx, ty;
        decode_tile(wk.tile, tilesX, tilesY, sk, tx, ty, i_n);
        i_c = wk.cb;
        i_ce = wk.ce;
        i_x = s2 ? 2 * tx * MT - 4 : tx * MT - 4;
        i_y = s2 ? 2 * ty * R - 1 : ty * R - 1;
      };
      auto issue = [&](uint32_t slot) {
        if (i_work >= numWork) return;
        const uint32_t bar = r_full + 8 * slot;
        if (dbg & 2) {
          mbar_arrive(bar);
        } else {
          mbar_arrive_expect_tx(bar, raw_bytes);
          tma_load_4d(raw_base + slot * raw_bytes, &tmx, i_x, i_y, 16 * i_c + 8 * i_h, i_n, bar);
        }
        if (++i_h < RPC) return;
        i_h = 0;
        if (++i_c >= i_ce) {
          i_work += gridDim.x;
          i_tile();
        }
      };
      if (issuer) {
        i_tile();
        for (int s = 0; s < RS; ++s) issue((uint32_t)s);
      }
      uint32_t as = 0, aph = 0, rs = 0, rph = 0;
      bool wrapped = false;
      for (int work = blockIdx.x; work < numWork; work += gridDim.x) {
        const Work wk = decode_work(work, sk, nChunks);
        for (int c = wk.cb; c < wk.ce; ++c) {
          unsigned char* a_st = smem + as * sm.a_stage;
          for (int h = 0; h < RPC; ++h) {
            mbar_wait(r_full + 8 * rs, rph);
            if (h == 0 && wrapped) mbar_wait(a_empty + 8 * as, aph ^ 1);
            const float* raw = reinterpret_cast<const float*>(smem + sm.raw_off + rs * raw_bytes);
            auto put = [&](int kc, int e, const float (&v)[8]) {
              if constexpr (P == 1) {
                *reinterpret_cast<uint4*>(a_st + (kc * E + e) * 16) =
                    make_uint4(bf16_pair(v[0], v[1]), bf16_pair(v[2], v[3]), bf16_pair(v[4], v[5]), bf16_pair(v[6], v[7]));
              } else {
                uint4 hi, lo;
                split_pair(v[0], v[1], hi.x, lo.x);
                split_pair(v[2], v[3], hi.y, lo.y);
                split_pair(v[4], v[5], hi.z, lo.z);
                split_pair(v[6], v[7], hi.w, lo.w);
                unsigned char* dst = a_st + (kc * E + e) * 16;
                *reinterpret_cast<uint4*>(dst) = hi;
                *reinterpret_cast<uint4*>(dst + sm.a_lo) = lo;
              }
            };
            if (s2) {
              constexpr int U = MT + 1;
              for (int u = pw * 32 + lane; u < (2 * R + 1) * U; u += NPROD * 32) {
                const int slot = u / U, j = u - slot * U;
                const float* s = raw + slot * RP + 2 * j + 2;
                float ve[8], vo[8];
#pragma unroll
                for (int jj = 0; jj < 8; ++jj) {
                  const float2 p2 = *reinterpret_cast<const float2*>(s + jj * CP);
                  ve[jj] = p2.x;
                  vo[jj] = p2.y;
                }
                put(h, slot * PW + MT + j, vo);
                if (j > 0) put(h, slot * PW + j - 1, ve);
              }
            } else {
#pragma unroll 2
              for (int t = pw; t < nItems; t += NPROD) {
                const int kc = one_plane ? 0 : (t & 1);
                const int e = (one_plane ? t : (t >> 1)) * 32 + lane;
                if (e >= E) continue;
                const int slot = e / (MT + 2), pe = e - slot * (MT + 2);
                const float* s = raw + 8 * kc * CP + slot * RP + pe + 3;
                float v[8];
#pragma unroll
                for (int jj = 0; jj < 8; ++jj) v[jj] = s[jj * CP];
                put(kc, e, v);
              }
            }
            const bool last = h == RPC - 1;
            if (last) asm volatile("fence.proxy.async.shared::cta;" ::: "memory");
            __syncwarp();
            if (lane == 0) {
              if (last) mbar_arrive(a_full + 8 * as);
              mbar_arrive(r_empty + 8 * rs);
            }
            if (issuer) {
              mbar_wait(r_empty + 8 * rs, rph);
              issue(rs);
            }
            __syncwarp();
            if (++rs == (uint32_t)RS) { rs = 0; rph ^= 1; }
          }
          if (++as == (uint32_t)AS) { as = 0; aph ^= 1; wrapped = true; }
        }
      }
      return;
    }
    int l_work = blockIdx.x, l_c = 0, l_kb = 0, l_x0 = 0, l_y0 = 0;
    const float* l_xn = x;
    int l_ce = nChunks;
    auto set_tile = [&]() {
      const Work wk = decode_work(l_work, sk, nChunks);
      l_c = wk.cb;
      l_ce = wk.ce;
      int tx, ty, n;
      decode_tile(wk.tile, tilesX, tilesY, sk, tx, ty, n);
      l_x0 = tx * MT - (ext ? 1 : 0);
      l_y0 = ty * R - (ext ? 1 : 0);
      l_xn = x + (size_t)n * x_bs;
    };
    auto advance = [&]() {
      if (++l_kb < nb) return true;
      l_kb = 0;
      if (++l_c < l_ce) return true;
      l_work += gridDim.x;
      if (l_work >= numWork) return false;
      set_tile();
      return true;
    };
    const bool s2 = stride == 2, wide = !s2 && dil >= R;
    const int ymul = s2 ? 2 : 1, ya = s2 ? -1 : -dil, yb = wide ? dil : 0, yc = wide ? 1 : 0, yd = wide ? 0 : 1;
    const int xa = s2 ? 0 : -dil;
    const uint32_t planeu = (uint32_t)plane;
    auto load_batch = [&](float (&v)[BATCH][8]) {
      const float* xc = l_xn + (size_t)(16 * l_c) * plane;
      const int ybase = ymul * l_y0 + ya, xbase = ymul * l_x0 + xa;
#pragma unroll
      for (int b = 0; b < BATCH; ++b) {
        const int t = pw + (l_kb * BATCH + b) * NPROD;
        const int kc = one_plane ? 0 : (t & 1);
        const int e = (one_plane ? t : (t >> 1)) * 32 + lane;
        const int slot = (int)__umulhi((uint32_t)e, pw_magic), pe = e - slot * PW;
        int y = ybase + yb * (slot >> 1) + yc * (slot & 1) + yd * slot;
        const int q = (s2 && pe >= MT) ? 1 : 0;
        int xx = xbase + ymul * (pe - q * MT) - q;
        if (ext == 2) {
          y = y >= 0 ? band_map(y, H) : -1;
          xx = xx >= 0 ? band_map(xx, W) : -1;
        }
        const bool ok = t < nItems && e < E && (unsigned)y < (unsigned)H && (unsigned)xx < (unsigned)W && !(dbg & 2);
        const int c0 = 16 * l_c + 8 * kc;
        uint32_t off = (uint32_t)(8 * kc) * planeu + (ok ? (uint32_t)(y * W + xx) : 0u);
        if (c0 + 8 <= Cin) {
#pragma unroll
          for (int jj = 0; jj < 8; ++jj) {
            v[b][jj] = ok ? __ldg(xc + off) : 0.f;
            off += planeu;
          }
        } else {
#pragma unroll
          for (int jj = 0; jj < 8; ++jj) {
            v[b][jj] = (ok && c0 + jj < Cin) ? __ldg(xc + off) : 0.f;
            off += planeu;
          }
        }
      }
    };
    uint32_t as = 0, aph = 0;
    bool wrapped = false;
    auto store_batch = [&](int kb, const float (&v)[BATCH][8]) {
      if (kb == 0 && wrapped) mbar_wait(a_empty + 8 * as, aph ^ 1);
      unsigned char* a_st = smem + as * sm.a_stage;
#pragma unroll
      for (int b = 0; b < BATCH; ++b) {
        const int t = pw + (kb * BATCH + b) * NPROD;
        const int kc = one_plane ? 0 : (t & 1);
        const int e = (one_plane ? t : (t >> 1)) * 32 + lane;
        if (t < nItems && e < E) {
          if constexpr (P == 1) {
            *reinterpret_cast<uint4*>(a_st + (kc * E + e) * 16) = make_uint4(
                bf16_pair(v[b][0], v[b][1]), bf16_pair(v[b][2], v[b][3]), bf16_pair(v[b][4], v[b][5]), bf16_pair(v[b][6], v[b][7]));
          } else {
            uint4 hi, lo;
            split_pair(v[b][0], v[b][1], hi.x, lo.x);
            split_pair(v[b][2], v[b][3], hi.y, lo.y);
            split_pair(v[b][4], v[b][5], hi.z, lo.z);
            split_pair(v[b][6], v[b][7], hi.w, lo.w);
            unsigned char* dst = a_st + (kc * E + e) * 16;
            *reinterpret_cast<uint4*>(dst) = hi;
            *reinterpret_cast<uint4*>(dst + sm.a_lo) = lo;
          }
        }
      }
      if (kb == nb - 1) {
        asm volatile("fence.proxy.async.shared::cta;" ::: "memory");
        __syncwarp();
        if (lane == 0) mbar_arrive(a_full + 8 * as);
        if (++as == (uint32_t)AS) { as = 0; aph ^= 1; wrapped = true; }
      }
    };
    float va[BATCH][8], vb[BATCH][8];
    set_tile();
    load_batch(va);
    int s_kb = 0;
    for (;;) {
      bool more = advance();
      if (more) load_batch(vb);
      store_batch(s_kb, va);
      if (!more) break;
      s_kb = l_kb;
      more = advance();
      if (more) load_batch(va);
      store_batch(s_kb, vb);
      if (!more) break;
      s_kb = l_kb;
    }
  }
}

long long conv3x3_wgmma_packed_bytes(int Cin, int Cout) {
  return (long long)((Cin + 15) / 16) * 9 * 64 * um::cout_pad(Cout);
}

int conv3x3_wgmma_pack(const float* weight, unsigned char* packed, int Cin, int Cout, cudaStream_t st) {
  const int CoutP = um::cout_pad(Cout), nChunks16 = (Cin + 15) / 16;
  const long long total = (long long)nChunks16 * 9 * CoutP * 8;
  long long blocks = (total + 255) / 256;
  if (blocks > 4096) blocks = 4096;
  conv3x3_pack_wgmma_kernel<<<(unsigned)blocks, 256, 0, st>>>(weight, packed, Cin, Cout, CoutP, nChunks16);
  return check_launch("conv3x3_pack_wgmma_kernel");
}

template <int TERMS>
__global__ void conv3x3_wgmma_reduce_kernel(um::SplitK sk, um::SplitDev xs, int RN, const float* __restrict__ bias,
                                            float* __restrict__ out, long long out_bs, int Cout, int OH, int OW, float slope,
                                            int out_mode_arg) {
  const int out_mode = out_mode_arg & 0xff, lin_prefix = out_mode_arg >> 8;
  const long long total = (long long)RN * Cout * sk.rh * OW;
  const int F = Cout >> 2;
  for (long long i = (long long)blockIdx.x * blockDim.x + threadIdx.x; i < total; i += (long long)gridDim.x * blockDim.x) {
    float s = 0.f;
    for (int p = 0; p < sk.k; ++p) s += sk.ws[(size_t)p * (size_t)sk.part_stride + (size_t)i];
    const int x = (int)(i % OW), y = sk.y_lo + (int)((i / OW) % sk.rh), f = (int)((i / ((long long)OW * sk.rh)) % Cout);
    const int n = sk.n_lo + (int)(i / ((long long)OW * sk.rh * Cout));
    if (out_mode == 0) {
      const float b = bias ? __ldg(bias + f) : 0.f;
      const float v = leaky(s + b, f < lin_prefix ? 1.f : slope);
      if (xs.out != nullptr && f >= lin_prefix)
        sa::put_one<TERMS == 1 ? 1 : 2>(xs.out, xs.out_Cg, (long long)OH * OW, n, xs.out_c0 + f - lin_prefix, (long long)y * OW + x, v);
      else
        out[(size_t)n * out_bs + ((size_t)f * OH + y) * OW + x] = v;
    } else {
      const int ph = f / F, ff = f - ph * F;
      const float b = bias ? __ldg(bias + ff) : 0.f;
      out[(size_t)n * out_bs + ((size_t)ff * (2 * OH) + (2 * y + (ph >> 1))) * (2 * OW) + 2 * x + (ph & 1)] = leaky(s + b, slope);
    }
  }
}

static um::SplitK plan_split(int N, int Cin, int H, int W, int Cout, int stride, int dil, int grid_cap) {
  using namespace um;
  (void)dil;
  const int ns = cout_pad(Cout) > 128 ? 2 : 1;
  SplitK sk = {1, 0, 0, 0, 0, 0, nullptr, 0u, 0u, 3, ns};
  const int OH = (H - 1) / stride + 1, OW = (W - 1) / stride + 1, nChunks = (Cin + 15) / 16;
  const int MT = tile_width(OW, stride);
  const int tilesX = (OW + MT - 1) / MT, tilesY = (OH + R - 1) / R;
  const long long tiles = (long long)N * tilesX * tilesY;
  sk.from = (int)tiles;
  const int mode = tuning().conv_splitk;
  if (!mode || tiles >= (1 << 29)) return sk;
  const int sms = grid_cap > 0 && grid_cap < kNumSMs ? grid_cap : kNumSMs;
  const int kcap = mode > 1 ? mode : 32;
  if (2 * tiles * ns <= sms) {
    int k = (int)(sms / (tiles * ns));
    if (k > nChunks / 3) k = nChunks / 3;
    if (k > 8) k = 8;
    if (k > kcap) k = kcap;
    if (k >= 2) {
      sk.k = k; sk.from = 0; sk.n_lo = 0; sk.y_lo = 0; sk.rh = OH;
    }
  } else if (ns == 1 && tiles > sms) {
    const long long rounds = tiles / sms;
    long long tail = tiles - rounds * sms;
    tail = (tail + tilesX - 1) / tilesX * tilesX;
    int k = tail > 0 ? (int)(sms / tail) : 0;
    if (k > nChunks / 2) k = nChunks / 2;
    if (k > kcap) k = kcap;
    if (tail > 0 && tail <= (long long)tilesX * tilesY && rounds <= 12 && k >= 2 && nChunks >= 16 && Cout > 64) {
      sk.k = k; sk.from = (int)(tiles - tail); sk.n_lo = N - 1;
      sk.y_lo = (int)((sk.from / tilesX) % tilesY) * R;
      sk.rh = OH - sk.y_lo;
    }
  }
  if (sk.k > 1) sk.part_stride = (long long)(N - sk.n_lo) * Cout * sk.rh * OW;
  return sk;
}

long long conv3x3_wgmma_workspace_bytes(int N, int Cin, int H, int W, int Cout, int stride, int dil) {
  const um::SplitK sk = plan_split(N, Cin, H, W, Cout, stride, dil, tuning().conv_grid_cap);
  return sk.k > 1 ? sk.k * sk.part_stride * 4 : 0;
}

int conv3x3_wgmma_launch(const float* x, long long x_bs, const unsigned char* wpack, const float* bias, float* out,
                         long long out_bs, int N, int Cin, int H, int W, int Cout, int stride, int dil, int out_mode,
                         float slope, cudaStream_t st, int ext, float* ws, long long ws_bytes, const SplitIO& sio) {
  using namespace um;
  const int terms = (out_mode & MFN_CONV_BF16) ? 1 : 3;
  out_mode &= ~MFN_CONV_BF16;
  const int grow = ext == 2 ? 8 : 2 * ext;
  const int OH = stride == 2 ? (H - 1) / 2 + 1 : H + grow, OW = stride == 2 ? (W - 1) / 2 + 1 : W + grow;
  const int MT = tile_width(OW, stride);
  SplitDev xs = {0, 0, 0, nullptr, 0, 0};
  CUtensorMap tmx;
  memset(&tmx, 0, sizeof tmx);
  if (sio.in != nullptr) {
    if (stride != 1 || ext != 0 || sio.in_c0 % 16 != 0 || (dil >= R && dil % 2 != 0) || !aligned(sio.in, 16)) return -1;
    EncodeTiledFn fn = encode_tiled_fn();
    if (fn == nullptr) return fail(MFN_ERR_UNSUPPORTED, "cuTensorMapEncodeTiled is not available from this driver");
    const int Cg = sa::groups(sio.in_C);
    const cuuint64_t dim[4] = {8, (cuuint64_t)W, (cuuint64_t)H, (cuuint64_t)N * (terms == 1 ? 1 : 2) * Cg};
    const cuuint64_t strides[3] = {16, (cuuint64_t)W * 16, (cuuint64_t)W * H * 16};
    const cuuint32_t box[4] = {8, (cuuint32_t)row_pitch(MT, 1, dil), (cuuint32_t)(dil < R ? n_slots(1, dil) : R), dil < R ? 2u : 1u};
    const cuuint32_t es[4] = {1, 1, 1, 1};
    const CUresult r = fn(&tmx, CU_TENSOR_MAP_DATA_TYPE_BFLOAT16, 4, const_cast<void*>(sio.in), dim, strides, box, es,
                          CU_TENSOR_MAP_INTERLEAVE_NONE, CU_TENSOR_MAP_SWIZZLE_NONE, CU_TENSOR_MAP_L2_PROMOTION_L2_256B,
                          CU_TENSOR_MAP_FLOAT_OOB_FILL_NONE);
    if (r != CUDA_SUCCESS) return fail(MFN_ERR_UNSUPPORTED, "cuTensorMapEncodeTiled failed (CUresult %d)", (int)r);
    xs.in = 1;
    xs.in_g0 = sio.in_c0 / 8;
    xs.in_Cg = Cg;
  }
  if (sio.out != nullptr) {
    const int lp = out_mode >> 8;
    if ((out_mode & 0xff) != 0 || ext != 0 || sio.out_c0 % 16 != 0 || (Cout - lp) % 16 != 0 || lp % 2 != 0 ||
        sio.out_c0 + Cout - lp > sio.out_C || !aligned(sio.out, 16))
      return -1;
    xs.out = static_cast<unsigned char*>(sio.out);
    xs.out_Cg = sa::groups(sio.out_C);
    xs.out_c0 = sio.out_c0;
  }
  if (Cout > 256 || (stride != 1 && !(stride == 2 && dil == 1))) return -1;
  if (ext != 0 && !((ext == 1 || ext == 2) && stride == 1 && dil == 1 && out_mode == 0)) return -1;
  if ((out_mode >> 8) != 0 && (out_mode & 0xff) != 0) return -1;
  const int CoutP = um::cout_pad(Cout), nChunks = (Cin + 15) / 16;
  const int E = n_slots(stride, dil) * row_pitch(MT, stride, dil);
  const int as_wide = tuning().conv_as == 2 ? 2 : 3;
  const bool staged = (out_mode & 0xff) == 0 && ext == 0 &&
                      (xs.out != nullptr ? (out_mode >> 8) == 0 : OW % 4 == 0 && out_bs % 4 == 0 && aligned(out, 16)) &&
                      smem_map(E, CoutP, as_wide, STG_BYTES, terms).WS >= 2;
  int raw = 0;
  const bool raw_geometry = stride == 1 ? dil == 1 && MT == MT_WIDE : MT == MT_NARROW && OW > MT_NARROW;
  if (sio.in == nullptr && tuning().conv_tma_in && raw_geometry && ext == 0 && W % 4 == 0 && x_bs % 4 == 0 &&
      aligned(x, 16)) {
    raw = raw_stage_bytes(n_slots(stride, 1), MT, stride);
    if (smem_map(E, CoutP, as_wide, staged ? STG_BYTES : 0, terms, raw, raw_ring_max(stride)).WS < 3) raw = 0;
  }
  if (raw) {
    EncodeTiledFn fn = encode_tiled_fn();
    if (fn == nullptr) return fail(MFN_ERR_UNSUPPORTED, "cuTensorMapEncodeTiled is not available from this driver");
    const cuuint64_t dim[4] = {(cuuint64_t)W, (cuuint64_t)H, (cuuint64_t)Cin, (cuuint64_t)N};
    const cuuint64_t strides[3] = {(cuuint64_t)W * 4, (cuuint64_t)W * H * 4, (cuuint64_t)x_bs * 4};
    const cuuint32_t box[4] = {(cuuint32_t)raw_pitch(MT, stride), (cuuint32_t)n_slots(stride, 1),
                               (cuuint32_t)raw_channels(stride), 1};
    const cuuint32_t es[4] = {1, 1, 1, 1};
    const CUresult r = fn(&tmx, CU_TENSOR_MAP_DATA_TYPE_FLOAT32, 4, const_cast<float*>(x), dim, strides, box, es,
                          CU_TENSOR_MAP_INTERLEAVE_NONE, CU_TENSOR_MAP_SWIZZLE_NONE, CU_TENSOR_MAP_L2_PROMOTION_L2_256B,
                          CU_TENSOR_MAP_FLOAT_OOB_FILL_NONE);
    if (r != CUDA_SUCCESS) return fail(MFN_ERR_UNSUPPORTED, "cuTensorMapEncodeTiled failed (CUresult %d)", (int)r);
    xs.in = 2;
  }
  const SmemMap sm = smem_map(E, CoutP, as_wide, staged ? STG_BYTES : 0, terms, raw, raw_ring_max(stride));
  if (sm.WS < 2 || E * 16 > 0x3FFF * 16) return -1;
  if ((long long)H * W >= (1LL << 27)) return -1;
  const int tilesX = (OW + MT - 1) / MT, tilesY = (OH + R - 1) / R;
  const int ns = CoutP > 128 ? 2 : 1;
  SplitK sk = {1, 0, 0, 0, 0, 0, nullptr, 0u, 0u, 3, ns};
  if (ws != nullptr && ext == 0) {
    sk = plan_split(N, Cin, H, W, Cout, stride, dil, tuning().conv_grid_cap);
    if (sk.k > 1 && ws_bytes < sk.k * sk.part_stride * 4) sk.k = 1;
    sk.ws = ws;
  }
  const long long tiles = (long long)N * tilesX * tilesY;
  if (tiles * ns >= (1LL << 30)) return -1;
  sk.as_wide = as_wide;
  sk.stg = staged ? STG_BYTES : 0;
  if (sk.k <= 1) sk.from = (int)tiles;
  {
    const unsigned long long tp = (unsigned long long)tilesX * tilesY;
    if ((unsigned long long)tiles * tp < (1ull << 32) && tp * tilesX < (1ull << 32)) {
      sk.magic_tp = (uint32_t)(((1ull << 32) + tp - 1) / tp);
      sk.magic_tx = tilesX == 1 ? 0u : (uint32_t)(((1ull << 32) + tilesX - 1) / tilesX);
    }
    if (tp == 1) sk.magic_tp = 0;
  }
  const long long numWork = (sk.from + (tiles - sk.from) * sk.k) * ns;
  const int cap = tuning().conv_grid_cap > 0 ? tuning().conv_grid_cap : kNumSMs;
  const unsigned grid = (unsigned)(numWork < cap ? numWork : cap);
  const char* name = terms == 3 ? "conv3x3_wgmma_kernel<CoutP=256>" : "conv3x3_wgmma_kernel<CoutP=256,bf16>";
  auto launch = [&](auto mt) -> cudaError_t {
    constexpr int M = decltype(mt)::value;
    static SmemOptIn opt[8], opt1[8];
    cudaError_t e = cudaSuccess;
    if (terms == 3) {
      e = ensure_dyn_smem(conv3x3_wgmma_kernel<32, true, 9, 3, M>, sm.total, opt[0]);
      if (e == cudaSuccess) e = ensure_dyn_smem(conv3x3_wgmma_kernel<64, true, 9, 3, M>, sm.total, opt[1]);
      if (e == cudaSuccess) e = ensure_dyn_smem(conv3x3_wgmma_kernel<96, true, 3, 3, M>, sm.total, opt[2]);
      if (e == cudaSuccess) e = ensure_dyn_smem(conv3x3_wgmma_kernel<128, true, 3, 3, M>, sm.total, opt[3]);
      if (e == cudaSuccess) e = ensure_dyn_smem(conv3x3_wgmma_kernel<80, false, 1, 3, M>, sm.total, opt[4]);
      if (e == cudaSuccess) e = ensure_dyn_smem(conv3x3_wgmma_kernel<96, false, 1, 3, M>, sm.total, opt[5]);
      if (e == cudaSuccess) e = ensure_dyn_smem(conv3x3_wgmma_kernel<112, false, 1, 3, M>, sm.total, opt[6]);
      if (e == cudaSuccess) e = ensure_dyn_smem(conv3x3_wgmma_kernel<128, false, 1, 3, M>, sm.total, opt[7]);
    } else {
      e = ensure_dyn_smem(conv3x3_wgmma_kernel<16, true, 9, 1, M>, sm.total, opt1[0]);
      if (e == cudaSuccess) e = ensure_dyn_smem(conv3x3_wgmma_kernel<32, true, 9, 1, M>, sm.total, opt1[1]);
      if (e == cudaSuccess) e = ensure_dyn_smem(conv3x3_wgmma_kernel<48, true, 3, 1, M>, sm.total, opt1[2]);
      if (e == cudaSuccess) e = ensure_dyn_smem(conv3x3_wgmma_kernel<64, true, 3, 1, M>, sm.total, opt1[3]);
      if (e == cudaSuccess) e = ensure_dyn_smem(conv3x3_wgmma_kernel<80, false, 1, 1, M>, sm.total, opt1[4]);
      if (e == cudaSuccess) e = ensure_dyn_smem(conv3x3_wgmma_kernel<96, false, 1, 1, M>, sm.total, opt1[5]);
      if (e == cudaSuccess) e = ensure_dyn_smem(conv3x3_wgmma_kernel<112, false, 1, 1, M>, sm.total, opt1[6]);
      if (e == cudaSuccess) e = ensure_dyn_smem(conv3x3_wgmma_kernel<128, false, 1, 1, M>, sm.total, opt1[7]);
    }
    if (e != cudaSuccess) return e;
#define MFN_WGMMA_LAUNCH(NW_, FOLD_, TPS_, TERMS_)                                                                      \
  conv3x3_wgmma_kernel<NW_, FOLD_, TPS_, TERMS_, M><<<grid, NTHREADS, sm.total, st>>>(                                 \
      x, x_bs, wpack, bias, out, out_bs, Cin, H, W, OH, OW, Cout, CoutP, nChunks, slope, tilesX, tilesY, (int)numWork, \
      stride, dil, out_mode, ext, sk, xs, tmx, tuning().conv_dbg)
    if (terms == 3) {
      switch (CoutP) {
        case 16: MFN_WGMMA_LAUNCH(32, true, 9, 3); name = "conv3x3_wgmma_kernel<CoutP=16,fold>"; break;
        case 32: MFN_WGMMA_LAUNCH(64, true, 9, 3); name = "conv3x3_wgmma_kernel<CoutP=32,fold>"; break;
        case 48: MFN_WGMMA_LAUNCH(96, true, 3, 3); name = "conv3x3_wgmma_kernel<CoutP=48,fold>"; break;
        case 64: MFN_WGMMA_LAUNCH(128, true, 3, 3); name = "conv3x3_wgmma_kernel<CoutP=64,fold>"; break;
        case 80: MFN_WGMMA_LAUNCH(80, false, 1, 3); name = "conv3x3_wgmma_kernel<CoutP=80>"; break;
        case 96: MFN_WGMMA_LAUNCH(96, false, 1, 3); name = "conv3x3_wgmma_kernel<CoutP=96>"; break;
        case 112: MFN_WGMMA_LAUNCH(112, false, 1, 3); name = "conv3x3_wgmma_kernel<CoutP=112>"; break;
        case 128: MFN_WGMMA_LAUNCH(128, false, 1, 3); name = "conv3x3_wgmma_kernel<CoutP=128>"; break;
        default: MFN_WGMMA_LAUNCH(128, false, 1, 3);
      }
    } else {
      switch (CoutP) {
        case 16: MFN_WGMMA_LAUNCH(16, true, 9, 1); name = "conv3x3_wgmma_kernel<CoutP=16,fold,bf16>"; break;
        case 32: MFN_WGMMA_LAUNCH(32, true, 9, 1); name = "conv3x3_wgmma_kernel<CoutP=32,fold,bf16>"; break;
        case 48: MFN_WGMMA_LAUNCH(48, true, 3, 1); name = "conv3x3_wgmma_kernel<CoutP=48,fold,bf16>"; break;
        case 64: MFN_WGMMA_LAUNCH(64, true, 3, 1); name = "conv3x3_wgmma_kernel<CoutP=64,fold,bf16>"; break;
        case 80: MFN_WGMMA_LAUNCH(80, false, 1, 1); name = "conv3x3_wgmma_kernel<CoutP=80,bf16>"; break;
        case 96: MFN_WGMMA_LAUNCH(96, false, 1, 1); name = "conv3x3_wgmma_kernel<CoutP=96,bf16>"; break;
        case 112: MFN_WGMMA_LAUNCH(112, false, 1, 1); name = "conv3x3_wgmma_kernel<CoutP=112,bf16>"; break;
        case 128: MFN_WGMMA_LAUNCH(128, false, 1, 1); name = "conv3x3_wgmma_kernel<CoutP=128,bf16>"; break;
        default: MFN_WGMMA_LAUNCH(128, false, 1, 1);
      }
    }
#undef MFN_WGMMA_LAUNCH
    return cudaSuccess;
  };
  const cudaError_t e = MT == MT_NARROW ? launch(std::integral_constant<int, MT_NARROW>{})
                                        : launch(std::integral_constant<int, MT_WIDE>{});
  if (e != cudaSuccess) return fail((int)e, "cudaFuncSetAttribute(conv3x3_wgmma_kernel): %s", cudaGetErrorString(e));
  const int rc = check_launch(name);
  if (rc != 0 || sk.k <= 1) return rc;
  const long long total = sk.part_stride;
  long long blocks = (total + 255) / 256;
  if (blocks > 4 * kNumSMs) blocks = 4 * kNumSMs;
  if (terms == 3) {
    conv3x3_wgmma_reduce_kernel<3><<<(unsigned)blocks, 256, 0, st>>>(sk, xs, N - sk.n_lo, bias, out, out_bs, Cout, OH, OW, slope, out_mode);
    return check_launch("conv3x3_wgmma_reduce_kernel");
  }
  conv3x3_wgmma_reduce_kernel<1><<<(unsigned)blocks, 256, 0, st>>>(sk, xs, N - sk.n_lo, bias, out, out_bs, Cout, OH, OW, slope, out_mode);
  return check_launch("conv3x3_wgmma_reduce_kernel<bf16>");
}

}
```

maskflownet_b200/csrc/mma_tiles.cuh:

```cuda
#pragma once
#include <cuda_bf16.h>

#include "common.cuh"
#include "ptx.cuh"

namespace mfn {
namespace c3 {
constexpr int TW = 32, HX = 4, HWP = TW + 2 * HX;
constexpr int PXB = 64;
constexpr int NTHREADS = 256;
constexpr int WSTAGES = 3;

__host__ __device__ constexpr int cout_pad(int cout) { return cout <= 32 ? 32 : (cout <= 64 ? 64 : (cout <= 96 ? 96 : 128)); }
}

long long conv3x3_sync_packed_bytes(int Cin, int Cout);
long long conv3x3_wgmma_packed_bytes(int Cin, int Cout);
int conv3x3_wgmma_pack(const float* weight, unsigned char* packed, int Cin, int Cout, cudaStream_t st);
struct SplitIO {
  const void* in = nullptr;
  int in_C = 0, in_c0 = 0;
  void* out = nullptr;
  int out_C = 0, out_c0 = 0;
};
int conv3x3_wgmma_launch(const float* x, long long x_bs, const unsigned char* wpack, const float* bias, float* out,
                        long long out_bs, int N, int Cin, int H, int W, int Cout, int stride, int dil, int out_mode,
                        float slope, cudaStream_t st, int ext = 0, float* ws = nullptr, long long ws_bytes = 0,
                        const SplitIO& sio = SplitIO());
typedef CUresult (*EncodeTiledFn)(CUtensorMap*, CUtensorMapDataType, cuuint32_t, void*, const cuuint64_t*, const cuuint64_t*,
                                  const cuuint32_t*, const cuuint32_t*, CUtensorMapInterleave, CUtensorMapSwizzle,
                                  CUtensorMapL2promotion, CUtensorMapFloatOOBfill);
EncodeTiledFn encode_tiled_fn();
long long conv3x3_wgmma_workspace_bytes(int N, int Cin, int H, int W, int Cout, int stride, int dil);

}
```

Baseline: 820.7.

## Add four-row tall tiles to the wgmma conv3x3 kernel for narrow output channels

Adds a tile-height template parameter so each consumer warpgroup computes two output rows instead of one, used for small Cout (16/32), behind a new conv_tall tuning knob that is on by default. Taller tiles reuse each staged weight tap across more output pixels and share halo rows, cutting weight and input traffic per output. In exchange it doubles the accumulator registers and shrinks the raw staging channels and epilogue staging buffer, which may reduce pipeline depth or occupancy. A tile-plan query API is also exposed.

```diff
diff --git a/include/maskflow_b200.h b/include/maskflow_b200.h
--- a/include/maskflow_b200.h
+++ b/include/maskflow_b200.h
@@ -122,6 +122,8 @@
                                    float* out, long long out_batch_stride, int N, int Cin, int H, int W, int Cout,
                                    int stride, int dilation, int out_mode, float leaky_slope, void* stream);
 MFN_API long long mfn_conv3x3_workspace_bytes(int N, int Cin, int H, int W, int Cout, int stride, int dilation);
+MFN_API int mfn_conv3x3_tile_plan(int N, int Cin, int H, int W, int Cout, int stride, int dilation, int bf16, int* rows,
+                                  int* smem_bytes);
 MFN_API int mfn_conv3x3_forward_ws(const float* x, long long x_batch_stride, const void* packed_weight, const float* bias,
                                    float* out, long long out_batch_stride, int N, int Cin, int H, int W, int Cout,
                                    int stride, int dilation, int out_mode, float leaky_slope, void* workspace,
diff --git a/maskflownet_b200/_lib.py b/maskflownet_b200/_lib.py
--- a/maskflownet_b200/_lib.py
+++ b/maskflownet_b200/_lib.py
@@ -35,6 +35,7 @@
     "mfn_flow_to_color": [_f, _f, _f, _i, _i, _i, _fl, _i, _f],
     "mfn_flow_consistency": [_f, _f, _f, _f, _i, _i, _i, _fl, _fl, _f],
     "mfn_interpolate_frames_workspace_bytes": [_i, _i, _i],
+    "mfn_conv3x3_tile_plan": [_i] * 8 + [_f, _f],
     "mfn_interpolate_frames": [_f] * 8 + [_ll, _i, _i, _i, _f, _i, _fl, _f],
     "mfn_warp_mask_backward_det": [_f] * 14 + [_i] * 5 + [_fl, _fl, _fl, _i, _f, _ll, _f],
     "mfn_deformable_conv_backward_det": [_f] * 8 + [_i] * 6 + [_f, _ll, _f],
diff --git a/maskflownet_b200/csrc/api.cu b/maskflownet_b200/csrc/api.cu
--- a/maskflownet_b200/csrc/api.cu
+++ b/maskflownet_b200/csrc/api.cu
@@ -53,6 +53,7 @@
   else if (!strcmp(key, "conv_splitk")) mfn::tuning().conv_splitk = value;
   else if (!strcmp(key, "conv_narrow")) mfn::tuning().conv_narrow = value;
   else if (!strcmp(key, "conv_tma_in")) mfn::tuning().conv_tma_in = value;
+  else if (!strcmp(key, "conv_tall")) mfn::tuning().conv_tall = value;
   else if (!strcmp(key, "corr_rb_twb")) mfn::tuning().corr_rb_twb = value;
   else if (!strcmp(key, "corr_rb_rows")) mfn::tuning().corr_rb_rows = value;
   else if (!strcmp(key, "corr_tma")) mfn::tuning().corr_tma = value;
diff --git a/maskflownet_b200/csrc/common.cuh b/maskflownet_b200/csrc/common.cuh
--- a/maskflownet_b200/csrc/common.cuh
+++ b/maskflownet_b200/csrc/common.cuh
@@ -25,6 +25,7 @@
   int conv_splitk = 1;
   int conv_narrow = 1;
   int conv_tma_in = 1;
+  int conv_tall = 1;
   int corr_rb_twb = 0;
   int corr_rb_rows = 0;
   int corr_tma = 1;
diff --git a/maskflownet_b200/csrc/conv3x3.cu b/maskflownet_b200/csrc/conv3x3.cu
--- a/maskflownet_b200/csrc/conv3x3.cu
+++ b/maskflownet_b200/csrc/conv3x3.cu
@@ -294,6 +294,17 @@
                                       void* stream) {
   return mfn_conv3x3_forward_ws(x, x_batch_stride, packed_weight, bias, out, out_batch_stride, N, Cin, H, W, Cout, stride,
                                 dilation, out_mode, leaky_slope, nullptr, 0, stream);
+}
+
+extern "C" int mfn_conv3x3_tile_plan(int N, int Cin, int H, int W, int Cout, int stride, int dilation, int bf16,
+                                     int* rows, int* smem_bytes) {
+  using namespace mfn;
+  if (rows == nullptr || smem_bytes == nullptr) return fail(MFN_ERR_INVALID_ARG, "mfn_conv3x3_tile_plan: null pointer");
+  if (N <= 0 || Cin <= 0 || H <= 0 || W <= 0 || Cout <= 0 || Cout > 256 || dilation < 1 ||
+      !(stride == 1 || (stride == 2 && dilation == 1)))
+    return fail(MFN_ERR_INVALID_ARG, "mfn_conv3x3_tile_plan: unsupported shape");
+  conv3x3_wgmma_tile_plan(N, Cin, H, W, Cout, stride, dilation, bf16, rows, smem_bytes);
+  return MFN_OK;
 }
 
 extern "C" long long mfn_conv3x3_workspace_bytes(int N, int Cin, int H, int W, int Cout, int stride, int dilation) {
diff --git a/maskflownet_b200/csrc/conv3x3_wgmma.cu b/maskflownet_b200/csrc/conv3x3_wgmma.cu
--- a/maskflownet_b200/csrc/conv3x3_wgmma.cu
+++ b/maskflownet_b200/csrc/conv3x3_wgmma.cu
@@ -11,6 +11,7 @@
   return tuning().conv_narrow && (OW <= MT_NARROW || (stride == 2 && tuning().conv_tma_in)) ? MT_NARROW : MT_WIDE;
 }
 constexpr int R = 2;
+constexpr int R_TALL = 4;
 constexpr int NTHREADS = 384;
 constexpr int NCONS = 8;
 constexpr int NPROD = 3;
@@ -19,21 +20,23 @@
 constexpr int BATCH = 6;
 constexpr int BAR_BYTES = 1024;
 
-__host__ __device__ inline int n_slots(int stride, int dil) { return stride == 2 ? 2 * R + 1 : (dil >= R ? 3 * R : R + 2 * dil); }
+__host__ __device__ inline int n_slots(int stride, int dil, int rt = R) {
+  return stride == 2 ? 2 * rt + 1 : (dil >= rt ? 3 * rt : rt + 2 * dil);
+}
 __host__ __device__ inline int row_pitch(int mt, int stride, int dil) { return stride == 2 ? 2 * mt + 1 : mt + 2 * dil; }
-__host__ __device__ inline int slot_of(int r, int ky, int stride, int dil) {
-  return stride == 2 ? 2 * r + ky : (dil >= R ? ky * R + r : r + ky * dil);
+__host__ __device__ inline int slot_of(int r, int ky, int stride, int dil, int rt = R) {
+  return stride == 2 ? 2 * r + ky : (dil >= rt ? ky * rt + r : r + ky * dil);
 }
 __host__ __device__ inline int tap_xoff(int mt, int kx, int stride, int dil) {
   return stride == 2 ? (kx == 1 ? 0 : (kx == 0 ? mt : mt + 1)) : kx * dil;
 }
 __host__ __device__ inline int band_map(int v, int n) { return v < n ? v : (v == n + 2 ? 0 : (v == n + 5 ? n - 1 : -1)); }
 __host__ __device__ inline int raw_pitch(int mt, int stride) { return stride == 2 ? 2 * mt + 4 : mt + 8; }
-__host__ __device__ inline int raw_channels(int stride) { return stride == 2 ? 8 : 16; }
-__host__ __device__ inline int raw_stage_bytes(int nslots, int mt, int stride) {
-  return raw_channels(stride) * nslots * raw_pitch(mt, stride) * 4;
-}
-__host__ __device__ inline int raw_ring_max(int stride) { return stride == 2 ? MAX_RS : 2; }
+__host__ __device__ inline int raw_channels(int stride, int rt = R) { return stride == 2 || rt == R_TALL ? 8 : 16; }
+__host__ __device__ inline int raw_stage_bytes(int nslots, int mt, int stride, int rt = R) {
+  return raw_channels(stride, rt) * nslots * raw_pitch(mt, stride) * 4;
+}
+__host__ __device__ inline int raw_ring_max(int stride, int rt = R) { return raw_channels(stride, rt) == 8 ? MAX_RS : 2; }
 __host__ __device__ inline int cout_pad(int cout) { return cout <= 128 ? (cout + 15) / 16 * 16 : 256; }
 __host__ __device__ inline bool fold_hi_lo(int CoutP) { return CoutP <= 64; }
 __host__ __device__ inline int taps_per_stage(int CoutP) { return CoutP <= 32 ? 9 : (CoutP <= 64 ? 3 : 1); }
@@ -187,8 +190,10 @@
 };
 constexpr int STG_CH = 32, SPITCH = MT_WIDE + 4;
 constexpr int STG_BYTES = R * STG_CH * SPITCH * 4;
+constexpr int STG_CH_TALL = 16;
+constexpr int STG_BYTES_TALL = R * STG_CH_TALL * SPITCH * 4;
 __host__ __device__ inline SmemMap smem_map(int E, int CoutP, int as_wide = 3, int stg = 0, int terms = 3, int raw = 0,
-                                            int rs_max = 2) {
+                                            int rs_max = 2, int rs_min = 2) {
   SmemMap m;
   m.a_lo = 2 * E * 16;
   m.a_stage = terms == 1 ? m.a_lo : 2 * m.a_lo;
@@ -199,7 +204,7 @@
   if (raw) {
     const int raw_off = (2 * m.a_stage + 127) / 128 * 128;
     m.RS = rs_max;
-    while (m.RS > 2 && budget - raw_off - m.RS * raw < 3 * m.w_stage) --m.RS;
+    while (m.RS > rs_min && budget - raw_off - m.RS * raw < 3 * m.w_stage) --m.RS;
     budget -= m.RS * raw + (raw_off - 2 * m.a_stage);
   }
   if (raw)
@@ -250,7 +255,7 @@
   }
 }
 
-template <int NW, bool FOLD, int TPS, int TERMS, int MT>
+template <int NW, bool FOLD, int TPS, int TERMS, int MT, int RT>
 __global__ void __launch_bounds__(um::NTHREADS, 1)
     conv3x3_wgmma_kernel(const float* __restrict__ x, long long x_bs, const unsigned char* __restrict__ wpack,
                          const float* __restrict__ bias_arg, float* __restrict__ out_base, long long out_bs, int Cin, int H, int W,
@@ -260,15 +265,17 @@
   using namespace um;
   static_assert(TERMS == 1 || TERMS == 3, "one or three products per multiply-add");
   static_assert(MT == MT_WIDE || MT == MT_NARROW, "128- or 64-pixel tile rows");
+  static_assert(RT == R || RT == R_TALL, "2- or 4-row tiles");
   constexpr bool FOLD_ACC = FOLD && TERMS == 3;
   constexpr int P = TERMS == 1 ? 1 : 2;
   constexpr int NCOL = FOLD_ACC ? NW / 2 : NW;
   constexpr int MB = MT / 64;
+  constexpr int RW = RT / R;
   const int out_mode_k = out_mode_arg & 0xff, lin_prefix_k = out_mode_arg >> 8;
   extern __shared__ __align__(128) unsigned char smem[];
-  const int nslots = n_slots(stride, dil), PW = row_pitch(MT, stride, dil), E = nslots * PW;
-  const SmemMap sm = smem_map(E, CoutP, sk.as_wide, sk.stg, TERMS, xs.in == 2 ? raw_stage_bytes(nslots, MT, stride) : 0,
-                              raw_ring_max(stride));
+  const int nslots = n_slots(stride, dil, RT), PW = row_pitch(MT, stride, dil), E = nslots * PW;
+  const SmemMap sm = smem_map(E, CoutP, sk.as_wide, sk.stg, TERMS, xs.in == 2 ? raw_stage_bytes(nslots, MT, stride, RT) : 0,
+                              raw_ring_max(stride, RT), RT == R_TALL ? 1 : 2);
   const int AS = sm.AS, WS = sm.WS, RS = sm.RS;
   const uint32_t s_base = smem_u32(smem);
   const uint32_t bar0 = s_base + sm.bar_off;
@@ -302,7 +309,8 @@
     uint32_t a_off[9];
 #pragma unroll
     for (int tap = 0; tap < 9; ++tap)
-      a_off[tap] = (uint32_t)(slot_of(r, tap / 3, stride, dil) * PW + tap_xoff(MT, tap % 3, stride, dil));
+      a_off[tap] = (uint32_t)(slot_of(RW * r, tap / 3, stride, dil, RT) * PW + tap_xoff(MT, tap % 3, stride, dil));
+    const uint32_t a_row = (uint32_t)((stride == 2 ? 2 : 1) * PW);
     const uint64_t dh_a = desc_hi(a_lbo, 128u), dh_b = desc_hi(b_lbo, 128u);
     uint32_t as = 0, aph = 0, ws = 0, wph = 0;
     const uint32_t a_lo16 = (uint32_t)sm.a_lo >> 4, a_stage16 = (uint32_t)sm.a_stage >> 4, s_base16 = s_base >> 4;
@@ -316,13 +324,13 @@
       }
       rel_w = rel_a = -1;
     };
-    float acc[MB][NW / 2];
+    float acc[RW * MB][NW / 2];
     for (int work = blockIdx.x; work < numWork; work += gridDim.x) {
       const Work wk = decode_work(work, sk, nChunks);
       const int cb = wk.cb, ce = wk.ce;
       const uint32_t b_nh16 = (uint32_t)(wk.nh * NCOL);
 #pragma unroll
-      for (int mh = 0; mh < MB; ++mh) fence_acc(acc[mh]);
+      for (int mh = 0; mh < RW * MB; ++mh) fence_acc(acc[mh]);
       if (dbg & 8) {
         for (int c = cb; c < ce; ++c) {
           mbar_wait(a_full + 8 * as, aph);
@@ -349,8 +357,8 @@
           const uint32_t sc = (tap == 0 && c == cb) ? 0u : 1u;
           wgmma_fence();
 #pragma unroll
-          for (int mh = 0; mh < MB; ++mh) {
-            const uint32_t a16 = a_st16 + a_off[tap] + (uint32_t)(64 * mh);
+          for (int mh = 0; mh < RW * MB; ++mh) {
+            const uint32_t a16 = a_st16 + a_off[tap] + (uint32_t)(mh / MB) * a_row + (uint32_t)(64 * (mh % MB));
             const uint64_t a_hi = dh_a | (uint64_t)a16, a_lo = dh_a | (uint64_t)(a16 + a_lo16);
             if constexpr (TERMS == 1) {
               wgmma_bf16<NW>(acc[mh], a_hi, b_hi, sc);
@@ -376,7 +384,7 @@
       }
       wgmma_wait<0>();
 #pragma unroll
-      for (int mh = 0; mh < MB; ++mh) fence_acc(acc[mh]);
+      for (int mh = 0; mh < RW * MB; ++mh) fence_acc(acc[mh]);
       release();
 
       int tx, ty, n;
@@ -389,123 +397,126 @@
       float* const out = partial ? sk.ws + (size_t)wk.part * (size_t)sk.part_stride + (size_t)(n - sk.n_lo) * Cout * oplane0 -
                                        (size_t)sk.y_lo * OW
                                  : out_base + (size_t)n * out_bs;
-      const int y = ty * R + r;
       const int F = Cout >> 2;
       const size_t oplane2 = (size_t)(2 * OH) * (2 * OW);
-      if (y < OH && !(dbg & 4) && sk.stg && !partial) {
-        constexpr int SCH = NCOL % STG_CH == 0 ? STG_CH : 16;
-        float* const stg = reinterpret_cast<float*>(smem + sm.stg_off) + r * STG_CH * SPITCH;
-        const int t = wq * 32 + lane;
-        const int x0 = tx * MT;
-        const uint32_t seg = (uint32_t)((OW - x0 < MT ? OW - x0 : MT) * 4);
-        if (xs.out != nullptr) {
-          unsigned char* const sst = reinterpret_cast<unsigned char*>(stg);
-#pragma unroll
+#pragma unroll
+      for (int rr = 0; rr < RW; ++rr) {
+        const int y = ty * RT + RW * r + rr;
+        if (y < OH && !(dbg & 4) && sk.stg && !partial) {
+          constexpr int SCH = RT == R_TALL ? STG_CH_TALL : (NCOL % STG_CH == 0 ? STG_CH : 16);
+          float* const stg = reinterpret_cast<float*>(smem + sm.stg_off) + r * SCH * SPITCH;
+          const int t = wq * 32 + lane;
+          const int x0 = tx * MT;
+          const uint32_t seg = (uint32_t)((OW - x0 < MT ? OW - x0 : MT) * 4);
+          if (xs.out != nullptr) {
+            unsigned char* const sst = reinterpret_cast<unsigned char*>(stg);
+  #pragma unroll
+            for (int pc = 0; pc < NCOL / SCH; ++pc) {
+              if (t < SCH * P / 8) bulk_wait_read();
+              named_bar_sync(1 + r, 128);
+  #pragma unroll
+              for (int jj = 0; jj < SCH / 8; ++jj) {
+                const int j = pc * (SCH / 8) + jj;
+                const int f = wk.nh * NCOL + 8 * j + 2 * (lane & 3);
+                const float b0 = (bias != nullptr && f < Cout) ? __ldg(bias + f) : 0.f;
+                const float b1 = (bias != nullptr && f + 1 < Cout) ? __ldg(bias + f + 1) : 0.f;
+                unsigned char* const row = sst + (P * jj * MT + 16 * wq + (lane >> 2)) * 16 + (lane & 3) * 4;
+  #pragma unroll
+                for (int mh = 0; mh < MB; ++mh)
+  #pragma unroll
+                  for (int h = 0; h < 2; ++h) {
+                    const int i = 4 * j + 2 * h;
+                    float v0 = acc[rr * MB + mh][i], v1 = acc[rr * MB + mh][i + 1];
+                    if constexpr (FOLD_ACC) {
+                      v0 += acc[rr * MB + mh][i + NW / 4];
+                      v1 += acc[rr * MB + mh][i + 1 + NW / 4];
+                    }
+                    unsigned char* const e = row + (64 * mh + 8 * h) * 16;
+                    if constexpr (TERMS == 1) {
+                      *reinterpret_cast<uint32_t*>(e) = bf16_pair(leaky(v0 + b0, slope), leaky(v1 + b1, slope));
+                    } else {
+                      uint32_t hi, lo;
+                      split_pair(leaky(v0 + b0, slope), leaky(v1 + b1, slope), hi, lo);
+                      *reinterpret_cast<uint32_t*>(e) = hi;
+                      *reinterpret_cast<uint32_t*>(e + MT * 16) = lo;
+                    }
+                  }
+              }
+              asm volatile("fence.proxy.async.shared::cta;" ::: "memory");
+              named_bar_sync(1 + r, 128);
+              const int f = wk.nh * NCOL + pc * SCH + 8 * (t >> (P - 1));
+              if (t < SCH * P / 8 && f < Cout) {
+                const long long dst = sa::entry<P>(n, t & (P - 1), (xs.out_c0 + f) >> 3, (long long)y * OW + x0, xs.out_Cg,
+                                                   oplane0);
+                bulk_s2g(xs.out + dst, smem_u32(sst + t * MT * 16), seg * 4);
+                bulk_commit();
+              }
+            }
+          } else
+  #pragma unroll
           for (int pc = 0; pc < NCOL / SCH; ++pc) {
-            if (t < SCH * P / 8) bulk_wait_read();
+            if (t < SCH) bulk_wait_read();
             named_bar_sync(1 + r, 128);
-#pragma unroll
+  #pragma unroll
             for (int jj = 0; jj < SCH / 8; ++jj) {
               const int j = pc * (SCH / 8) + jj;
-              const int f = wk.nh * NCOL + 8 * j + 2 * (lane & 3);
-              const float b0 = (bias != nullptr && f < Cout) ? __ldg(bias + f) : 0.f;
-              const float b1 = (bias != nullptr && f + 1 < Cout) ? __ldg(bias + f + 1) : 0.f;
-              unsigned char* const row = sst + (P * jj * MT + 16 * wq + (lane >> 2)) * 16 + (lane & 3) * 4;
-#pragma unroll
-              for (int mh = 0; mh < MB; ++mh)
-#pragma unroll
-                for (int h = 0; h < 2; ++h) {
-                  const int i = 4 * j + 2 * h;
-                  float v0 = acc[mh][i], v1 = acc[mh][i + 1];
-                  if constexpr (FOLD_ACC) {
-                    v0 += acc[mh][i + NW / 4];
-                    v1 += acc[mh][i + 1 + NW / 4];
+  #pragma unroll
+              for (int e = 0; e < 2; ++e) {
+                const int f = wk.nh * NCOL + 8 * j + 2 * (lane & 3) + e;
+                const float b = (bias != nullptr && f < Cout) ? __ldg(bias + f) : 0.f;
+                const float sl = f < lin_prefix ? 1.f : slope;
+                float* const row = stg + (8 * jj + 2 * (lane & 3) + e) * SPITCH + 16 * wq + (lane >> 2);
+  #pragma unroll
+                for (int mh = 0; mh < MB; ++mh)
+  #pragma unroll
+                  for (int h = 0; h < 2; ++h) {
+                    const int i = 4 * j + 2 * h + e;
+                    float v = acc[rr * MB + mh][i];
+                    if constexpr (FOLD_ACC) v += acc[rr * MB + mh][i + NW / 4];
+                    row[64 * mh + 8 * h] = leaky(v + b, sl);
                   }
-                  unsigned char* const e = row + (64 * mh + 8 * h) * 16;
-                  if constexpr (TERMS == 1) {
-                    *reinterpret_cast<uint32_t*>(e) = bf16_pair(leaky(v0 + b0, slope), leaky(v1 + b1, slope));
-                  } else {
-                    uint32_t hi, lo;
-                    split_pair(leaky(v0 + b0, slope), leaky(v1 + b1, slope), hi, lo);
-                    *reinterpret_cast<uint32_t*>(e) = hi;
-                    *reinterpret_cast<uint32_t*>(e + MT * 16) = lo;
-                  }
-                }
+              }
             }
             asm volatile("fence.proxy.async.shared::cta;" ::: "memory");
             named_bar_sync(1 + r, 128);
-            const int f = wk.nh * NCOL + pc * SCH + 8 * (t >> (P - 1));
-            if (t < SCH * P / 8 && f < Cout) {
-              const long long dst = sa::entry<P>(n, t & (P - 1), (xs.out_c0 + f) >> 3, (long long)y * OW + x0, xs.out_Cg,
-                                                 oplane0);
-              bulk_s2g(xs.out + dst, smem_u32(sst + t * MT * 16), seg * 4);
+            const int f = wk.nh * NCOL + pc * SCH + t;
+            if (t < SCH && f < Cout) {
+              bulk_s2g(out + (size_t)f * oplane0 + (size_t)y * OW + x0, smem_u32(stg + t * SPITCH), seg);
               bulk_commit();
             }
           }
-        } else
-#pragma unroll
-        for (int pc = 0; pc < NCOL / SCH; ++pc) {
-          if (t < SCH) bulk_wait_read();
-          named_bar_sync(1 + r, 128);
-#pragma unroll
-          for (int jj = 0; jj < SCH / 8; ++jj) {
-            const int j = pc * (SCH / 8) + jj;
-#pragma unroll
-            for (int e = 0; e < 2; ++e) {
-              const int f = wk.nh * NCOL + 8 * j + 2 * (lane & 3) + e;
-              const float b = (bias != nullptr && f < Cout) ? __ldg(bias + f) : 0.f;
-              const float sl = f < lin_prefix ? 1.f : slope;
-              float* const row = stg + (8 * jj + 2 * (lane & 3) + e) * SPITCH + 16 * wq + (lane >> 2);
-#pragma unroll
-              for (int mh = 0; mh < MB; ++mh)
-#pragma unroll
-                for (int h = 0; h < 2; ++h) {
+        } else if (y < OH && !(dbg & 4)) {
+  #pragma unroll
+          for (int mh = 0; mh < MB; ++mh) {
+  #pragma unroll
+            for (int h = 0; h < 2; ++h) {
+              const int xx = tx * MT + 64 * mh + 16 * wq + (lane >> 2) + 8 * h;
+              if (xx >= OW) continue;
+  #pragma unroll
+              for (int j = 0; j < NCOL / 8; ++j) {
+  #pragma unroll
+                for (int e = 0; e < 2; ++e) {
                   const int i = 4 * j + 2 * h + e;
-                  float v = acc[mh][i];
-                  if constexpr (FOLD_ACC) v += acc[mh][i + NW / 4];
-                  row[64 * mh + 8 * h] = leaky(v + b, sl);
-                }
-            }
-          }
-          asm volatile("fence.proxy.async.shared::cta;" ::: "memory");
-          named_bar_sync(1 + r, 128);
-          const int f = wk.nh * NCOL + pc * SCH + t;
-          if (t < SCH && f < Cout) {
-            bulk_s2g(out + (size_t)f * oplane0 + (size_t)y * OW + x0, smem_u32(stg + t * SPITCH), seg);
-            bulk_commit();
-          }
-        }
-      } else if (y < OH && !(dbg & 4)) {
-#pragma unroll
-        for (int mh = 0; mh < MB; ++mh) {
-#pragma unroll
-          for (int h = 0; h < 2; ++h) {
-            const int xx = tx * MT + 64 * mh + 16 * wq + (lane >> 2) + 8 * h;
-            if (xx >= OW) continue;
-#pragma unroll
-            for (int j = 0; j < NCOL / 8; ++j) {
-#pragma unroll
-              for (int e = 0; e < 2; ++e) {
-                const int i = 4 * j + 2 * h + e;
-                float v = acc[mh][i];
-                if constexpr (FOLD_ACC) v += acc[mh][i + NW / 4];
-                const int f = wk.nh * NCOL + 8 * j + 2 * (lane & 3) + e;
-                if (f >= Cout) continue;
-                if (xs.out != nullptr && !partial && f >= lin_prefix) {
-                  if (e == 0) {
-                    const float b0 = bias != nullptr ? __ldg(bias + f) : 0.f, b1 = bias != nullptr ? __ldg(bias + f + 1) : 0.f;
-                    float v1 = acc[mh][i + 1];
-                    if constexpr (FOLD_ACC) v1 += acc[mh][i + 1 + NW / 4];
-                    sa::put_pair<P>(xs.out, xs.out_Cg, oplane0, n, xs.out_c0 + f - lin_prefix, (size_t)y * OW + xx,
-                                 leaky(v + b0, slope), leaky(v1 + b1, slope));
+                  float v = acc[rr * MB + mh][i];
+                  if constexpr (FOLD_ACC) v += acc[rr * MB + mh][i + NW / 4];
+                  const int f = wk.nh * NCOL + 8 * j + 2 * (lane & 3) + e;
+                  if (f >= Cout) continue;
+                  if (xs.out != nullptr && !partial && f >= lin_prefix) {
+                    if (e == 0) {
+                      const float b0 = bias != nullptr ? __ldg(bias + f) : 0.f, b1 = bias != nullptr ? __ldg(bias + f + 1) : 0.f;
+                      float v1 = acc[rr * MB + mh][i + 1];
+                      if constexpr (FOLD_ACC) v1 += acc[rr * MB + mh][i + 1 + NW / 4];
+                      sa::put_pair<P>(xs.out, xs.out_Cg, oplane0, n, xs.out_c0 + f - lin_prefix, (size_t)y * OW + xx,
+                                   leaky(v + b0, slope), leaky(v1 + b1, slope));
+                    }
+                  } else if (out_mode == 0) {
+                    const float t = v + (bias != nullptr ? __ldg(bias + f) : 0.f);
+                    out[(size_t)f * oplane0 + (size_t)y * OW + xx] = leaky(t, f < lin_prefix ? 1.f : slope);
+                  } else {
+                    const int ph = f / F, ff = f - ph * F;
+                    const float t = v + (bias != nullptr ? __ldg(bias + ff) : 0.f);
+                    out[(size_t)ff * oplane2 + (size_t)(2 * y + (ph >> 1)) * (2 * OW) + 2 * xx + (ph & 1)] = leaky(t, slope);
                   }
-                } else if (out_mode == 0) {
-                  const float t = v + (bias != nullptr ? __ldg(bias + f) : 0.f);
-                  out[(size_t)f * oplane0 + (size_t)y * OW + xx] = leaky(t, f < lin_prefix ? 1.f : slope);
-                } else {
-                  const int ph = f / F, ff = f - ph * F;
-                  const float t = v + (bias != nullptr ? __ldg(bias + ff) : 0.f);
-                  out[(size_t)ff * oplane2 + (size_t)(2 * y + (ph >> 1)) * (2 * OW) + 2 * xx + (ph & 1)] = leaky(t, slope);
                 }
               }
             }
@@ -559,7 +570,7 @@
           const Work wk = decode_work(work, sk, nChunks);
           int tx, ty, n;
           decode_tile(wk.tile, tilesX, tilesY, sk, tx, ty, n);
-          const int x0 = tx * MT - dil, y0 = ty * R;
+          const int x0 = tx * MT - dil, y0 = ty * RT;
           const int gb = n * P * xs.in_Cg + xs.in_g0;
           for (int c = wk.cb; c < wk.ce; ++c) {
             if (wrapped) mbar_wait(a_empty + 8 * as, aph ^ 1);
@@ -569,20 +580,20 @@
             } else {
               mbar_arrive_expect_tx(bar, (uint32_t)sm.a_stage);
               const int g = gb + 2 * c;
-              if (dil < R) {
+              if (dil < RT) {
                 tma_load_4d(dst, &tmx, 0, x0, y0 - dil, g, bar);
                 if constexpr (P == 2) tma_load_4d(dst + (uint32_t)sm.a_lo, &tmx, 0, x0, y0 - dil, g + xs.in_Cg, bar);
               } else if constexpr (P == 1) {
 #pragma unroll 1
                 for (int k = 0; k < 6; ++k) {
                   const int ky = k >> 1, kc = k & 1;
-                  tma_load_4d(dst + (uint32_t)((kc * E + ky * R * PW) * 16), &tmx, 0, x0, y0 + (ky - 1) * dil, g + kc, bar);
+                  tma_load_4d(dst + (uint32_t)((kc * E + ky * RT * PW) * 16), &tmx, 0, x0, y0 + (ky - 1) * dil, g + kc, bar);
                 }
               } else {
 #pragma unroll 1
                 for (int k = 0; k < 12; ++k) {
                   const int ky = k >> 2, kc = (k >> 1) & 1, pl = k & 1;
-                  tma_load_4d(dst + (uint32_t)(pl * sm.a_lo + (kc * E + ky * R * PW) * 16), &tmx, 0, x0, y0 + (ky - 1) * dil,
+                  tma_load_4d(dst + (uint32_t)(pl * sm.a_lo + (kc * E + ky * RT * PW) * 16), &tmx, 0, x0, y0 + (ky - 1) * dil,
                               g + kc + pl * xs.in_Cg, bar);
                 }
               }
@@ -624,7 +635,8 @@
     if (xs.in == 2) {
       const bool s2 = stride == 2;
       const int RP = raw_pitch(MT, stride), CP = nslots * RP;
-      const int RPC = s2 && !one_plane ? 2 : 1;
+      const bool planes = raw_channels(stride, RT) == 8;
+      const int RPC = planes && !one_plane ? 2 : 1;
       const uint32_t raw_bytes = (uint32_t)sm.raw_stage, raw_base = s_base + (uint32_t)sm.raw_off;
       const bool issuer = warp == 9 && lane == 0;
       int i_work = blockIdx.x, i_c = 0, i_h = 0, i_ce = 0, i_x = 0, i_y = 0, i_n = 0;
@@ -636,7 +648,7 @@
         i_c = wk.cb;
         i_ce = wk.ce;
         i_x = s2 ? 2 * tx * MT - 4 : tx * MT - 4;
-        i_y = s2 ? 2 * ty * R - 1 : ty * R - 1;
+        i_y = s2 ? 2 * ty * RT - 1 : ty * RT - 1;
       };
       auto issue = [&](uint32_t slot) {
         if (i_work >= numWork) return;
@@ -685,7 +697,7 @@
             };
             if (s2) {
               constexpr int U = MT + 1;
-              for (int u = pw * 32 + lane; u < (2 * R + 1) * U; u += NPROD * 32) {
+              for (int u = pw * 32 + lane; u < nslots * U; u += NPROD * 32) {
                 const int slot = u / U, j = u - slot * U;
                 const float* s = raw + slot * RP + 2 * j + 2;
                 float ve[8], vo[8];
@@ -700,12 +712,12 @@
               }
             } else {
 #pragma unroll 2
-              for (int t = pw; t < nItems; t += NPROD) {
-                const int kc = one_plane ? 0 : (t & 1);
-                const int e = (one_plane ? t : (t >> 1)) * 32 + lane;
+              for (int t = pw; t < (planes ? G : nItems); t += NPROD) {
+                const int kc = planes ? h : (one_plane ? 0 : (t & 1));
+                const int e = (planes || one_plane ? t : (t >> 1)) * 32 + lane;
                 if (e >= E) continue;
                 const int slot = e / (MT + 2), pe = e - slot * (MT + 2);
-                const float* s = raw + 8 * kc * CP + slot * RP + pe + 3;
+                const float* s = raw + (planes ? 0 : 8 * kc * CP) + slot * RP + pe + 3;
                 float v[8];
 #pragma unroll
                 for (int jj = 0; jj < 8; ++jj) v[jj] = s[jj * CP];
@@ -741,7 +753,7 @@
       int tx, ty, n;
       decode_tile(wk.tile, tilesX, tilesY, sk, tx, ty, n);
       l_x0 = tx * MT - (ext ? 1 : 0);
-      l_y0 = ty * R - (ext ? 1 : 0);
+      l_y0 = ty * RT - (ext ? 1 : 0);
       l_xn = x + (size_t)n * x_bs;
     };
     auto advance = [&]() {
@@ -753,7 +765,7 @@
       set_tile();
       return true;
     };
-    const bool s2 = stride == 2, wide = !s2 && dil >= R;
+    const bool s2 = stride == 2, wide = !s2 && dil >= RT;
     const int ymul = s2 ? 2 : 1, ya = s2 ? -1 : -dil, yb = wide ? dil : 0, yc = wide ? 1 : 0, yd = wide ? 0 : 1;
     const int xa = s2 ? 0 : -dil;
     const uint32_t planeu = (uint32_t)plane;
@@ -766,7 +778,7 @@
         const int kc = one_plane ? 0 : (t & 1);
         const int e = (one_plane ? t : (t >> 1)) * 32 + lane;
         const int slot = (int)__umulhi((uint32_t)e, pw_magic), pe = e - slot * PW;
-        int y = ybase + yb * (slot >> 1) + yc * (slot & 1) + yd * slot;
+        int y = ybase + yb * (slot / RT) + yc * (slot % RT) + yd * slot;
         const int q = (s2 && pe >= MT) ? 1 : 0;
         int xx = xbase + ymul * (pe - q * MT) - q;
         if (ext == 2) {
@@ -922,9 +934,64 @@
   return sk;
 }
 
+static bool tall_candidate(int N, int Cin, int H, int W, int Cout, int stride, int dil, int ext, bool fp32_in, int OW) {
+  using namespace um;
+  return tuning().conv_tall && fp32_in && ext == 0 && dil == 1 && cout_pad(Cout) <= 32 && OW > MT_NARROW &&
+         plan_split(N, Cin, H, W, Cout, stride, dil, tuning().conv_grid_cap).k == 1;
+}
+struct TilePlan {
+  bool staged;
+  int raw;
+  um::SmemMap sm;
+};
+static TilePlan tile_plan(int rt, int MT, int E, int CoutP, int as_wide, int terms, bool stage_ok, bool raw_ok, int stride) {
+  using namespace um;
+  TilePlan p;
+  const int stg = rt == R_TALL ? STG_BYTES_TALL : STG_BYTES, rs_min = rt == R_TALL ? 1 : 2;
+  p.staged = stage_ok && smem_map(E, CoutP, as_wide, stg, terms).WS >= 2;
+  p.raw = 0;
+  if (raw_ok) {
+    p.raw = raw_stage_bytes(n_slots(stride, 1, rt), MT, stride, rt);
+    if (smem_map(E, CoutP, as_wide, p.staged ? stg : 0, terms, p.raw, raw_ring_max(stride, rt), rs_min).WS < 3) p.raw = 0;
+  }
+  p.sm = smem_map(E, CoutP, as_wide, p.staged ? stg : 0, terms, p.raw, raw_ring_max(stride, rt), rs_min);
+  return p;
+}
+
 long long conv3x3_wgmma_workspace_bytes(int N, int Cin, int H, int W, int Cout, int stride, int dil) {
   const um::SplitK sk = plan_split(N, Cin, H, W, Cout, stride, dil, tuning().conv_grid_cap);
   return sk.k > 1 ? sk.k * sk.part_stride * 4 : 0;
+}
+
+struct LaunchPlan {
+  int RT, E;
+  TilePlan tp;
+};
+static LaunchPlan launch_plan(int N, int Cin, int H, int W, int Cout, int stride, int dil, int ext, int OW, int MT, int terms,
+                              bool fp32_in, bool x_aligned, bool stage_ok) {
+  using namespace um;
+  const int CoutP = cout_pad(Cout), as_wide = tuning().conv_as == 2 ? 2 : 3;
+  const bool raw_geometry = stride == 1 ? dil == 1 && MT == MT_WIDE : MT == MT_NARROW && OW > MT_NARROW;
+  const bool raw_ok = fp32_in && tuning().conv_tma_in && raw_geometry && ext == 0 && x_aligned;
+  LaunchPlan lp;
+  lp.RT = R;
+  lp.E = n_slots(stride, dil) * row_pitch(MT, stride, dil);
+  lp.tp = tile_plan(R, MT, lp.E, CoutP, as_wide, terms, stage_ok, raw_ok, stride);
+  if (tall_candidate(N, Cin, H, W, Cout, stride, dil, ext, fp32_in, OW)) {
+    const int E4 = n_slots(stride, dil, R_TALL) * row_pitch(MT, stride, dil);
+    const TilePlan t4 = tile_plan(R_TALL, MT, E4, CoutP, as_wide, terms, stage_ok, raw_ok, stride);
+    if (t4.staged == lp.tp.staged && (t4.raw != 0) == (lp.tp.raw != 0) && t4.sm.WS >= 3) lp = {R_TALL, E4, t4};
+  }
+  return lp;
+}
+
+void conv3x3_wgmma_tile_plan(int N, int Cin, int H, int W, int Cout, int stride, int dil, int bf16, int* rows,
+                             int* smem_bytes) {
+  const int OW = (W - 1) / stride + 1;
+  const LaunchPlan lp = launch_plan(N, Cin, H, W, Cout, stride, dil, 0, OW, um::tile_width(OW, stride), bf16 ? 1 : 3, true,
+                                    W % 4 == 0, OW % 4 == 0);
+  *rows = lp.RT;
+  *smem_bytes = lp.tp.sm.total;
 }
 
 int conv3x3_wgmma_launch(const float* x, long long x_bs, const unsigned char* wpack, const float* bias, float* out,
@@ -969,25 +1036,22 @@
   if (ext != 0 && !((ext == 1 || ext == 2) && stride == 1 && dil == 1 && out_mode == 0)) return -1;
   if ((out_mode >> 8) != 0 && (out_mode & 0xff) != 0) return -1;
   const int CoutP = um::cout_pad(Cout), nChunks = (Cin + 15) / 16;
-  const int E = n_slots(stride, dil) * row_pitch(MT, stride, dil);
   const int as_wide = tuning().conv_as == 2 ? 2 : 3;
-  const bool staged = (out_mode & 0xff) == 0 && ext == 0 &&
-                      (xs.out != nullptr ? (out_mode >> 8) == 0 : OW % 4 == 0 && out_bs % 4 == 0 && aligned(out, 16)) &&
-                      smem_map(E, CoutP, as_wide, STG_BYTES, terms).WS >= 2;
-  int raw = 0;
-  const bool raw_geometry = stride == 1 ? dil == 1 && MT == MT_WIDE : MT == MT_NARROW && OW > MT_NARROW;
-  if (sio.in == nullptr && tuning().conv_tma_in && raw_geometry && ext == 0 && W % 4 == 0 && x_bs % 4 == 0 &&
-      aligned(x, 16)) {
-    raw = raw_stage_bytes(n_slots(stride, 1), MT, stride);
-    if (smem_map(E, CoutP, as_wide, staged ? STG_BYTES : 0, terms, raw, raw_ring_max(stride)).WS < 3) raw = 0;
-  }
+  const bool stage_ok = (out_mode & 0xff) == 0 && ext == 0 &&
+                        (xs.out != nullptr ? (out_mode >> 8) == 0 : OW % 4 == 0 && out_bs % 4 == 0 && aligned(out, 16));
+  const LaunchPlan lp = launch_plan(N, Cin, H, W, Cout, stride, dil, ext, OW, MT, terms, sio.in == nullptr,
+                                    W % 4 == 0 && x_bs % 4 == 0 && aligned(x, 16), stage_ok);
+  const int RT = lp.RT, E = lp.E;
+  const TilePlan& tp = lp.tp;
+  const bool staged = tp.staged;
+  const int raw = tp.raw;
   if (raw) {
     EncodeTiledFn fn = encode_tiled_fn();
     if (fn == nullptr) return fail(MFN_ERR_UNSUPPORTED, "cuTensorMapEncodeTiled is not available from this driver");
     const cuuint64_t dim[4] = {(cuuint64_t)W, (cuuint64_t)H, (cuuint64_t)Cin, (cuuint64_t)N};
     const cuuint64_t strides[3] = {(cuuint64_t)W * 4, (cuuint64_t)W * H * 4, (cuuint64_t)x_bs * 4};
-    const cuuint32_t box[4] = {(cuuint32_t)raw_pitch(MT, stride), (cuuint32_t)n_slots(stride, 1),
-                               (cuuint32_t)raw_channels(stride), 1};
+    const cuuint32_t box[4] = {(cuuint32_t)raw_pitch(MT, stride), (cuuint32_t)n_slots(stride, 1, RT),
+                               (cuuint32_t)raw_channels(stride, RT), 1};
     const cuuint32_t es[4] = {1, 1, 1, 1};
     const CUresult r = fn(&tmx, CU_TENSOR_MAP_DATA_TYPE_FLOAT32, 4, const_cast<float*>(x), dim, strides, box, es,
                           CU_TENSOR_MAP_INTERLEAVE_NONE, CU_TENSOR_MAP_SWIZZLE_NONE, CU_TENSOR_MAP_L2_PROMOTION_L2_256B,
@@ -995,10 +1059,10 @@
     if (r != CUDA_SUCCESS) return fail(MFN_ERR_UNSUPPORTED, "cuTensorMapEncodeTiled failed (CUresult %d)", (int)r);
     xs.in = 2;
   }
-  const SmemMap sm = smem_map(E, CoutP, as_wide, staged ? STG_BYTES : 0, terms, raw, raw_ring_max(stride));
+  const SmemMap sm = tp.sm;
   if (sm.WS < 2 || E * 16 > 0x3FFF * 16) return -1;
   if ((long long)H * W >= (1LL << 27)) return -1;
-  const int tilesX = (OW + MT - 1) / MT, tilesY = (OH + R - 1) / R;
+  const int tilesX = (OW + MT - 1) / MT, tilesY = (OH + RT - 1) / RT;
   const int ns = CoutP > 128 ? 2 : 1;
   SplitK sk = {1, 0, 0, 0, 0, 0, nullptr, 0u, 0u, 3, ns};
   if (ws != nullptr && ext == 0) {
@@ -1009,7 +1073,7 @@
   const long long tiles = (long long)N * tilesX * tilesY;
   if (tiles * ns >= (1LL << 30)) return -1;
   sk.as_wide = as_wide;
-  sk.stg = staged ? STG_BYTES : 0;
+  sk.stg = staged ? (RT == R_TALL ? STG_BYTES_TALL : STG_BYTES) : 0;
   if (sk.k <= 1) sk.from = (int)tiles;
   {
     const unsigned long long tp = (unsigned long long)tilesX * tilesY;
@@ -1023,64 +1087,86 @@
   const int cap = tuning().conv_grid_cap > 0 ? tuning().conv_grid_cap : kNumSMs;
   const unsigned grid = (unsigned)(numWork < cap ? numWork : cap);
   const char* name = terms == 3 ? "conv3x3_wgmma_kernel<CoutP=256>" : "conv3x3_wgmma_kernel<CoutP=256,bf16>";
-  auto launch = [&](auto mt) -> cudaError_t {
-    constexpr int M = decltype(mt)::value;
+  auto launch = [&](auto mt, auto rt) -> cudaError_t {
+    constexpr int M = decltype(mt)::value, RR = decltype(rt)::value;
     static SmemOptIn opt[8], opt1[8];
     cudaError_t e = cudaSuccess;
-    if (terms == 3) {
-      e = ensure_dyn_smem(conv3x3_wgmma_kernel<32, true, 9, 3, M>, sm.total, opt[0]);
-      if (e == cudaSuccess) e = ensure_dyn_smem(conv3x3_wgmma_kernel<64, true, 9, 3, M>, sm.total, opt[1]);
-      if (e == cudaSuccess) e = ensure_dyn_smem(conv3x3_wgmma_kernel<96, true, 3, 3, M>, sm.total, opt[2]);
-      if (e == cudaSuccess) e = ensure_dyn_smem(conv3x3_wgmma_kernel<128, true, 3, 3, M>, sm.total, opt[3]);
-      if (e == cudaSuccess) e = ensure_dyn_smem(conv3x3_wgmma_kernel<80, false, 1, 3, M>, sm.total, opt[4]);
-      if (e == cudaSuccess) e = ensure_dyn_smem(conv3x3_wgmma_kernel<96, false, 1, 3, M>, sm.total, opt[5]);
-      if (e == cudaSuccess) e = ensure_dyn_smem(conv3x3_wgmma_kernel<112, false, 1, 3, M>, sm.total, opt[6]);
-      if (e == cudaSuccess) e = ensure_dyn_smem(conv3x3_wgmma_kernel<128, false, 1, 3, M>, sm.total, opt[7]);
-    } else {
-      e = ensure_dyn_smem(conv3x3_wgmma_kernel<16, true, 9, 1, M>, sm.total, opt1[0]);
-      if (e == cudaSuccess) e = ensure_dyn_smem(conv3x3_wgmma_kernel<32, true, 9, 1, M>, sm.total, opt1[1]);
-      if (e == cudaSuccess) e = ensure_dyn_smem(conv3x3_wgmma_kernel<48, true, 3, 1, M>, sm.total, opt1[2]);
-      if (e == cudaSuccess) e = ensure_dyn_smem(conv3x3_wgmma_kernel<64, true, 3, 1, M>, sm.total, opt1[3]);
-      if (e == cudaSuccess) e = ensure_dyn_smem(conv3x3_wgmma_kernel<80, false, 1, 1, M>, sm.total, opt1[4]);
-      if (e == cudaSuccess) e = ensure_dyn_smem(conv3x3_wgmma_kernel<96, false, 1, 1, M>, sm.total, opt1[5]);
-      if (e == cudaSuccess) e = ensure_dyn_smem(conv3x3_wgmma_kernel<112, false, 1, 1, M>, sm.total, opt1[6]);
-      if (e == cudaSuccess) e = ensure_dyn_smem(conv3x3_wgmma_kernel<128, false, 1, 1, M>, sm.total, opt1[7]);
-    }
-    if (e != cudaSuccess) return e;
 #define MFN_WGMMA_LAUNCH(NW_, FOLD_, TPS_, TERMS_)                                                                      \
-  conv3x3_wgmma_kernel<NW_, FOLD_, TPS_, TERMS_, M><<<grid, NTHREADS, sm.total, st>>>(                                 \
+  conv3x3_wgmma_kernel<NW_, FOLD_, TPS_, TERMS_, M, RR><<<grid, NTHREADS, sm.total, st>>>(                             \
       x, x_bs, wpack, bias, out, out_bs, Cin, H, W, OH, OW, Cout, CoutP, nChunks, slope, tilesX, tilesY, (int)numWork, \
       stride, dil, out_mode, ext, sk, xs, tmx, tuning().conv_dbg)
-    if (terms == 3) {
-      switch (CoutP) {
-        case 16: MFN_WGMMA_LAUNCH(32, true, 9, 3); name = "conv3x3_wgmma_kernel<CoutP=16,fold>"; break;
-        case 32: MFN_WGMMA_LAUNCH(64, true, 9, 3); name = "conv3x3_wgmma_kernel<CoutP=32,fold>"; break;
-        case 48: MFN_WGMMA_LAUNCH(96, true, 3, 3); name = "conv3x3_wgmma_kernel<CoutP=48,fold>"; break;
-        case 64: MFN_WGMMA_LAUNCH(128, true, 3, 3); name = "conv3x3_wgmma_kernel<CoutP=64,fold>"; break;
-        case 80: MFN_WGMMA_LAUNCH(80, false, 1, 3); name = "conv3x3_wgmma_kernel<CoutP=80>"; break;
-        case 96: MFN_WGMMA_LAUNCH(96, false, 1, 3); name = "conv3x3_wgmma_kernel<CoutP=96>"; break;
-        case 112: MFN_WGMMA_LAUNCH(112, false, 1, 3); name = "conv3x3_wgmma_kernel<CoutP=112>"; break;
-        case 128: MFN_WGMMA_LAUNCH(128, false, 1, 3); name = "conv3x3_wgmma_kernel<CoutP=128>"; break;
-        default: MFN_WGMMA_LAUNCH(128, false, 1, 3);
-      }
+    if constexpr (RR == R_TALL) {
+      if (terms == 3) {
+        e = ensure_dyn_smem(conv3x3_wgmma_kernel<32, true, 9, 3, M, RR>, sm.total, opt[0]);
+        if (e == cudaSuccess) e = ensure_dyn_smem(conv3x3_wgmma_kernel<64, true, 9, 3, M, RR>, sm.total, opt[1]);
+      } else {
+        e = ensure_dyn_smem(conv3x3_wgmma_kernel<16, true, 9, 1, M, RR>, sm.total, opt1[0]);
+        if (e == cudaSuccess) e = ensure_dyn_smem(conv3x3_wgmma_kernel<32, true, 9, 1, M, RR>, sm.total, opt1[1]);
+      }
+      if (e != cudaSuccess) return e;
+      if (terms == 3) {
+        if (CoutP == 16) { MFN_WGMMA_LAUNCH(32, true, 9, 3); name = "conv3x3_wgmma_kernel<CoutP=16,fold>"; }
+        else { MFN_WGMMA_LAUNCH(64, true, 9, 3); name = "conv3x3_wgmma_kernel<CoutP=32,fold>"; }
+      } else {
+        if (CoutP == 16) { MFN_WGMMA_LAUNCH(16, true, 9, 1); name = "conv3x3_wgmma_kernel<CoutP=16,fold,bf16>"; }
+        else { MFN_WGMMA_LAUNCH(32, true, 9, 1); name = "conv3x3_wgmma_kernel<CoutP=32,fold,bf16>"; }
+      }
+      return cudaSuccess;
     } else {
-      switch (CoutP) {
-        case 16: MFN_WGMMA_LAUNCH(16, true, 9, 1); name = "conv3x3_wgmma_kernel<CoutP=16,fold,bf16>"; break;
-        case 32: MFN_WGMMA_LAUNCH(32, true, 9, 1); name = "conv3x3_wgmma_kernel<CoutP=32,fold,bf16>"; break;
-        case 48: MFN_WGMMA_LAUNCH(48, true, 3, 1); name = "conv3x3_wgmma_kernel<CoutP=48,fold,bf16>"; break;
-        case 64: MFN_WGMMA_LAUNCH(64, true, 3, 1); name = "conv3x3_wgmma_kernel<CoutP=64,fold,bf16>"; break;
-        case 80: MFN_WGMMA_LAUNCH(80, false, 1, 1); name = "conv3x3_wgmma_kernel<CoutP=80,bf16>"; break;
-        case 96: MFN_WGMMA_LAUNCH(96, false, 1, 1); name = "conv3x3_wgmma_kernel<CoutP=96,bf16>"; break;
-        case 112: MFN_WGMMA_LAUNCH(112, false, 1, 1); name = "conv3x3_wgmma_kernel<CoutP=112,bf16>"; break;
-        case 128: MFN_WGMMA_LAUNCH(128, false, 1, 1); name = "conv3x3_wgmma_kernel<CoutP=128,bf16>"; break;
-        default: MFN_WGMMA_LAUNCH(128, false, 1, 1);
-      }
+      if (terms == 3) {
+        e = ensure_dyn_smem(conv3x3_wgmma_kernel<32, true, 9, 3, M, RR>, sm.total, opt[0]);
+        if (e == cudaSuccess) e = ensure_dyn_smem(conv3x3_wgmma_kernel<64, true, 9, 3, M, RR>, sm.total, opt[1]);
+        if (e == cudaSuccess) e = ensure_dyn_smem(conv3x3_wgmma_kernel<96, true, 3, 3, M, RR>, sm.total, opt[2]);
+        if (e == cudaSuccess) e = ensure_dyn_smem(conv3x3_wgmma_kernel<128, true, 3, 3, M, RR>, sm.total, opt[3]);
+        if (e == cudaSuccess) e = ensure_dyn_smem(conv3x3_wgmma_kernel<80, false, 1, 3, M, RR>, sm.total, opt[4]);
+        if (e == cudaSuccess) e = ensure_dyn_smem(conv3x3_wgmma_kernel<96, false, 1, 3, M, RR>, sm.total, opt[5]);
+        if (e == cudaSuccess) e = ensure_dyn_smem(conv3x3_wgmma_kernel<112, false, 1, 3, M, RR>, sm.total, opt[6]);
+        if (e == cudaSuccess) e = ensure_dyn_smem(conv3x3_wgmma_kernel<128, false, 1, 3, M, RR>, sm.total, opt[7]);
+      } else {
+        e = ensure_dyn_smem(conv3x3_wgmma_kernel<16, true, 9, 1, M, RR>, sm.total, opt1[0]);
+        if (e == cudaSuccess) e = ensure_dyn_smem(conv3x3_wgmma_kernel<32, true, 9, 1, M, RR>, sm.total, opt1[1]);
+        if (e == cudaSuccess) e = ensure_dyn_smem(conv3x3_wgmma_kernel<48, true, 3, 1, M, RR>, sm.total, opt1[2]);
+        if (e == cudaSuccess) e = ensure_dyn_smem(conv3x3_wgmma_kernel<64, true, 3, 1, M, RR>, sm.total, opt1[3]);
+        if (e == cudaSuccess) e = ensure_dyn_smem(conv3x3_wgmma_kernel<80, false, 1, 1, M, RR>, sm.total, opt1[4]);
+        if (e == cudaSuccess) e = ensure_dyn_smem(conv3x3_wgmma_kernel<96, false, 1, 1, M, RR>, sm.total, opt1[5]);
+        if (e == cudaSuccess) e = ensure_dyn_smem(conv3x3_wgmma_kernel<112, false, 1, 1, M, RR>, sm.total, opt1[6]);
+        if (e == cudaSuccess) e = ensure_dyn_smem(conv3x3_wgmma_kernel<128, false, 1, 1, M, RR>, sm.total, opt1[7]);
+      }
+      if (e != cudaSuccess) return e;
+      if (terms == 3) {
+        switch (CoutP) {
+          case 16: MFN_WGMMA_LAUNCH(32, true, 9, 3); name = "conv3x3_wgmma_kernel<CoutP=16,fold>"; break;
+          case 32: MFN_WGMMA_LAUNCH(64, true, 9, 3); name = "conv3x3_wgmma_kernel<CoutP=32,fold>"; break;
+          case 48: MFN_WGMMA_LAUNCH(96, true, 3, 3); name = "conv3x3_wgmma_kernel<CoutP=48,fold>"; break;
+          case 64: MFN_WGMMA_LAUNCH(128, true, 3, 3); name = "conv3x3_wgmma_kernel<CoutP=64,fold>"; break;
+          case 80: MFN_WGMMA_LAUNCH(80, false, 1, 3); name = "conv3x3_wgmma_kernel<CoutP=80>"; break;
+          case 96: MFN_WGMMA_LAUNCH(96, false, 1, 3); name = "conv3x3_wgmma_kernel<CoutP=96>"; break;
+          case 112: MFN_WGMMA_LAUNCH(112, false, 1, 3); name = "conv3x3_wgmma_kernel<CoutP=112>"; break;
+          case 128: MFN_WGMMA_LAUNCH(128, false, 1, 3); name = "conv3x3_wgmma_kernel<CoutP=128>"; break;
+          default: MFN_WGMMA_LAUNCH(128, false, 1, 3);
+        }
+      } else {
+        switch (CoutP) {
+          case 16: MFN_WGMMA_LAUNCH(16, true, 9, 1); name = "conv3x3_wgmma_kernel<CoutP=16,fold,bf16>"; break;
+          case 32: MFN_WGMMA_LAUNCH(32, true, 9, 1); name = "conv3x3_wgmma_kernel<CoutP=32,fold,bf16>"; break;
+          case 48: MFN_WGMMA_LAUNCH(48, true, 3, 1); name = "conv3x3_wgmma_kernel<CoutP=48,fold,bf16>"; break;
+          case 64: MFN_WGMMA_LAUNCH(64, true, 3, 1); name = "conv3x3_wgmma_kernel<CoutP=64,fold,bf16>"; break;
+          case 80: MFN_WGMMA_LAUNCH(80, false, 1, 1); name = "conv3x3_wgmma_kernel<CoutP=80,bf16>"; break;
+          case 96: MFN_WGMMA_LAUNCH(96, false, 1, 1); name = "conv3x3_wgmma_kernel<CoutP=96,bf16>"; break;
+          case 112: MFN_WGMMA_LAUNCH(112, false, 1, 1); name = "conv3x3_wgmma_kernel<CoutP=112,bf16>"; break;
+          case 128: MFN_WGMMA_LAUNCH(128, false, 1, 1); name = "conv3x3_wgmma_kernel<CoutP=128,bf16>"; break;
+          default: MFN_WGMMA_LAUNCH(128, false, 1, 1);
+        }
+      }
+      return cudaSuccess;
     }
 #undef MFN_WGMMA_LAUNCH
-    return cudaSuccess;
   };
-  const cudaError_t e = MT == MT_NARROW ? launch(std::integral_constant<int, MT_NARROW>{})
-                                        : launch(std::integral_constant<int, MT_WIDE>{});
+  const cudaError_t e =
+      RT == R_TALL ? (MT == MT_NARROW ? launch(std::integral_constant<int, MT_NARROW>{}, std::integral_constant<int, R_TALL>{})
+                                      : launch(std::integral_constant<int, MT_WIDE>{}, std::integral_constant<int, R_TALL>{}))
+                   : (MT == MT_NARROW ? launch(std::integral_constant<int, MT_NARROW>{}, std::integral_constant<int, R>{})
+                                      : launch(std::integral_constant<int, MT_WIDE>{}, std::integral_constant<int, R>{}));
   if (e != cudaSuccess) return fail((int)e, "cudaFuncSetAttribute(conv3x3_wgmma_kernel): %s", cudaGetErrorString(e));
   const int rc = check_launch(name);
   if (rc != 0 || sk.k <= 1) return rc;
diff --git a/maskflownet_b200/csrc/mma_tiles.cuh b/maskflownet_b200/csrc/mma_tiles.cuh
--- a/maskflownet_b200/csrc/mma_tiles.cuh
+++ b/maskflownet_b200/csrc/mma_tiles.cuh
@@ -27,6 +27,8 @@
                         long long out_bs, int N, int Cin, int H, int W, int Cout, int stride, int dil, int out_mode,
                         float slope, cudaStream_t st, int ext = 0, float* ws = nullptr, long long ws_bytes = 0,
                         const SplitIO& sio = SplitIO());
+void conv3x3_wgmma_tile_plan(int N, int Cin, int H, int W, int Cout, int stride, int dil, int bf16, int* rows,
+                             int* smem_bytes);
 typedef CUresult (*EncodeTiledFn)(CUtensorMap*, CUtensorMapDataType, cuuint32_t, void*, const cuuint64_t*, const cuuint64_t*,
                                   const cuuint32_t*, const cuuint32_t*, CUtensorMapInterleave, CUtensorMapSwizzle,
                                   CUtensorMapL2promotion, CUtensorMapFloatOOBfill);
```

Result: no change. 828.6, median of 6 (+1.0%).
